# Wangshihu12/Voxel-SLAM

Hardware: AMD Instinct MI355X
Metric: local-BA iterations/sec (200k pts, W=10) (higher is better)
Workload: dtype f64

## Files before the change

voxel-slam_amd/csrc/vba_kernels_factor.hpp:

```cpp
#pragma once
#include <hip/hip_runtime.h>
#include "vba_eig3.hpp"

namespace vba {

struct FactorView {
  double *cl;
  double *fix;
  double *coe;
  double *eigval;
  double *eigvec;
  double *pcr;
  unsigned int *occ;
  int *tiles;
  int vs;
  int W;
};

__host__ __device__ inline int mask_bucket(unsigned int m, int nb) {
  constexpr int C[11][11] = {{1, 0, 0, 0, 0, 0, 0, 0, 0, 0, 0}, {1, 1, 0, 0, 0, 0, 0, 0, 0, 0, 0}, {1, 2, 1, 0, 0, 0, 0, 0, 0, 0, 0}, {1, 3, 3, 1, 0, 0, 0, 0, 0, 0, 0},
                             {1, 4, 6, 4, 1, 0, 0, 0, 0, 0, 0}, {1, 5, 10, 10, 5, 1, 0, 0, 0, 0, 0}, {1, 6, 15, 20, 15, 6, 1, 0, 0, 0, 0},
                             {1, 7, 21, 35, 35, 21, 7, 1, 0, 0, 0}, {1, 8, 28, 56, 70, 56, 28, 8, 1, 0, 0}, {1, 9, 36, 84, 126, 126, 84, 36, 9, 1, 0},
                             {1, 10, 45, 120, 210, 252, 210, 120, 45, 10, 1}};
  int p = 0;
  for (int b = 0; b < nb; b++) p += (m >> b) & 1u;
  int off = 0;
  for (int q = nb; q > p; q--) off += C[nb][q];
  int r = 0, k = 0;
  for (int b = 0; b < nb; b++)
    if ((m >> b) & 1u) { k++; r += C[b][k]; }
  return off + r;
}

__device__ __forceinline__ void jacobi_rot(double &app, double &aqq, double &apq, double &arp, double &arq,
                                           double &v0p, double &v0q, double &v1p, double &v1q, double &v2p, double &v2q,
                                           int sweep) {
  if (apq == 0.0) return;
  const double g = 100.0 * fabs(apq);
  if (fabs(app) + g == fabs(app) && fabs(aqq) + g == fabs(aqq)) { apq = 0.0; return; }
  const double a = 0.5 * (aqq - app);
  int ex;
  (void)frexp(fmax(fabs(a), fabs(apq)), &ex);
  const float af = (float)ldexp(a, -ex), bf = (float)ldexp(apq, -ex);
  const float tf = bf * __builtin_amdgcn_rcpf(fabsf(af) + __builtin_amdgcn_sqrtf(af * af + bf * bf));
  const double t = (af < 0.0f) ? -(double)tf : (double)tf;
  const double x = 1.0 + t * t;
  double c = __builtin_amdgcn_rsq(x);
  c = c * (1.5 - 0.5 * x * c * c);
  c = c * (1.5 - 0.5 * x * c * c);
  const double s = t * c;
  const double cc = c * c, ss = s * s, cs = c * s;
  const double npp = cc * app - 2.0 * cs * apq + ss * aqq;
  const double nqq = ss * app + 2.0 * cs * apq + cc * aqq;
  const double npq = cs * (app - aqq) + (cc - ss) * apq;
  app = npp; aqq = nqq; apq = npq;
  double x1 = arp, y1 = arq;
  arp = c * x1 - s * y1; arq = s * x1 + c * y1;
  x1 = v0p; y1 = v0q; v0p = c * x1 - s * y1; v0q = s * x1 + c * y1;
  x1 = v1p; y1 = v1q; v1p = c * x1 - s * y1; v1q = s * x1 + c * y1;
  x1 = v2p; y1 = v2q; v2p = c * x1 - s * y1; v2q = s * x1 + c * y1;
}

#define VBA_SWAP(a, b) { double _t = a; a = b; b = _t; }

__device__ __forceinline__ Eig3 eig3_jacobi_dev(double a00, double a01, double a02, double a11, double a12, double a22) {
  int e = 0;
  {
    const double s = fmax(fmax(fmax(fabs(a00), fabs(a11)), fabs(a22)), fmax(fmax(fabs(a01), fabs(a02)), fabs(a12)));
    if (s > 0.0 && s <= 1.7976931348623157e308) (void)frexp(s, &e);
  }
  a00 = ldexp(a00, -e); a01 = ldexp(a01, -e); a02 = ldexp(a02, -e); a11 = ldexp(a11, -e); a12 = ldexp(a12, -e); a22 = ldexp(a22, -e);
  double v00 = 1, v01 = 0, v02 = 0, v10 = 0, v11 = 1, v12 = 0, v20 = 0, v21 = 0, v22 = 1;
#pragma unroll 1
  for (int sweep = 0; sweep < 30; sweep++) {
    if (fabs(a01) + fabs(a02) + fabs(a12) == 0.0) break;
    jacobi_rot(a00, a11, a01, a02, a12, v00, v01, v10, v11, v20, v21, sweep);
    jacobi_rot(a00, a22, a02, a01, a12, v00, v02, v10, v12, v20, v22, sweep);
    jacobi_rot(a11, a22, a12, a01, a02, v01, v02, v11, v12, v21, v22, sweep);
  }
  if (a11 < a00) { VBA_SWAP(a00, a11); VBA_SWAP(v00, v01); VBA_SWAP(v10, v11); VBA_SWAP(v20, v21); }
  if (a22 < a00) { VBA_SWAP(a00, a22); VBA_SWAP(v00, v02); VBA_SWAP(v10, v12); VBA_SWAP(v20, v22); }
  if (a22 < a11) { VBA_SWAP(a11, a22); VBA_SWAP(v01, v02); VBA_SWAP(v11, v12); VBA_SWAP(v21, v22); }
  Eig3 o;
  o.w0 = ldexp(a00, e); o.w1 = ldexp(a11, e); o.w2 = ldexp(a22, e);
  o.v00 = v00; o.v01 = v01; o.v02 = v02; o.v10 = v10; o.v11 = v11; o.v12 = v12; o.v20 = v20; o.v21 = v21; o.v22 = v22;
  return o;
}

__device__ __forceinline__ void eig3_sym_dev(double a00, double a01, double a02, double a11, double a12, double a22,
                                             double &w0, double &w1, double &w2, double *V) {
  Eig3 o;
  if (!eig3_direct(a00, a01, a02, a11, a12, a22, o)) o = eig3_jacobi_dev(a00, a01, a02, a11, a12, a22);
  w0 = o.w0; w1 = o.w1; w2 = o.w2;
  V[0] = o.v00; V[1] = o.v01; V[2] = o.v02; V[3] = o.v10; V[4] = o.v11; V[5] = o.v12; V[6] = o.v20; V[7] = o.v21; V[8] = o.v22;
}

__global__ void k_aos_to_soa(FactorView f, int base, int n, const double *__restrict__ clusters, const double *__restrict__ fix,
                             const double *__restrict__ coe, const double *__restrict__ eig_val, const double *__restrict__ eig_vec,
                             const double *__restrict__ pcr_add) {
  const int W = f.W;
  const int per = 10 * W + 10 + 1 + 3 + 9 + 10;
  const long long tot = (long long)n * per;
  for (long long t = (long long)blockIdx.x * blockDim.x + threadIdx.x; t < tot; t += (long long)gridDim.x * blockDim.x) {
    const int a = (int)(t / per);
    int j = (int)(t % per);
    const int v = base + a;
    if (j < 10 * W) {
      const int i = j / 10, fld = j % 10;
      f.cl[((size_t)fld * W + i) * f.vs + v] = clusters[((size_t)a * W + i) * 10 + fld];
      continue;
    }
    j -= 10 * W;
    if (j < 10) { f.fix[(size_t)j * f.vs + v] = fix[(size_t)a * 10 + j]; continue; }
    j -= 10;
    if (j < 1) { f.coe[v] = coe[a]; continue; }
    j -= 1;
    if (j < 3) { f.eigval[(size_t)j * f.vs + v] = eig_val[(size_t)a * 3 + j]; continue; }
    j -= 3;
    if (j < 9) { f.eigvec[(size_t)j * f.vs + v] = eig_vec[(size_t)a * 9 + j]; continue; }
    j -= 9;
    f.pcr[(size_t)j * f.vs + v] = pcr_add[(size_t)a * 10 + j];
  }
}

__global__ void k_soa_to_aos_out(FactorView f, int n, double *__restrict__ eig_val, double *__restrict__ eig_vec, double *__restrict__ pcr_add) {
  const long long tot = (long long)n * 22;
  for (long long t = (long long)blockIdx.x * blockDim.x + threadIdx.x; t < tot; t += (long long)gridDim.x * blockDim.x) {
    const int v = (int)(t / 22);
    int j = (int)(t % 22);
    if (j < 3) { eig_val[(size_t)v * 3 + j] = f.eigval[(size_t)j * f.vs + v]; continue; }
    j -= 3;
    if (j < 9) { eig_vec[(size_t)v * 9 + j] = f.eigvec[(size_t)j * f.vs + v]; continue; }
    j -= 9;
    pcr_add[(size_t)v * 10 + j] = f.pcr[(size_t)j * f.vs + v];
  }
}

__global__ void k_factor_mask(FactorView f, int base, int n) {
  const int t = blockIdx.x * blockDim.x + threadIdx.x;
  if (t >= n) return;
  const int v = base + t;
  const size_t vs = (size_t)f.vs;
  unsigned int m = 0;
  for (int i = 0; i < f.W; i++) m |= (f.cl[((size_t)9 * f.W + i) * vs + v] != 0.0) ? (1u << i) : 0u;
  f.occ[v] = m;
}

__global__ void k_count_slots(FactorView f, int n, unsigned long long *out) {
  const long long tot = (long long)n * f.W;
  unsigned long long c = 0;
  for (long long t = (long long)blockIdx.x * blockDim.x + threadIdx.x; t < tot; t += (long long)gridDim.x * blockDim.x) {
    const int i = (int)(t / n), v = (int)(t % n);
    if (f.cl[((size_t)9 * f.W + i) * f.vs + v] != 0.0) c++;
  }
  if (c) atomicAdd(out, c);
}

__global__ __launch_bounds__(256) void k_calib_read8(const double *__restrict__ buf, double *__restrict__ sink) {
  const size_t nthr = (size_t)gridDim.x * blockDim.x, t = (size_t)blockIdx.x * blockDim.x + threadIdx.x;
  double acc = 0.0;
#pragma unroll
  for (int k = 0; k < 16; k++) acc += buf[t + (size_t)k * nthr];
  if (acc == 123.456) sink[0] = acc;
}

struct Cl10 { double p00, p10, p20, p11, p21, p22, v0, v1, v2, n; };
__device__ __forceinline__ Cl10 cluster_transform_exact(double c0, double c1, double c2, double c3, double c4, double c5, double v0, double v1, double v2, double n,
                                                        const double *R) {
#pragma clang fp contract(off)
  const double R0 = R[0], R1 = R[1], R2 = R[2], R3 = R[3], R4 = R[4], R5 = R[5], R6 = R[6], R7 = R[7], R8 = R[8];
  const double tx = R[9], ty = R[10], tz = R[11];
  const double rv0 = (R0 * v0 + R1 * v1) + R2 * v2, rv1 = (R3 * v0 + R4 * v1) + R5 * v2, rv2 = (R6 * v0 + R7 * v1) + R8 * v2;
  const double m00 = (R0 * c0 + R1 * c1) + R2 * c2, m01 = (R0 * c1 + R1 * c3) + R2 * c4, m02 = (R0 * c2 + R1 * c4) + R2 * c5;
  const double m10 = (R3 * c0 + R4 * c1) + R5 * c2, m11 = (R3 * c1 + R4 * c3) + R5 * c4, m12 = (R3 * c2 + R4 * c4) + R5 * c5;
  const double m20 = (R6 * c0 + R7 * c1) + R8 * c2, m21 = (R6 * c1 + R7 * c3) + R8 * c4, m22 = (R6 * c2 + R7 * c4) + R8 * c5;
  Cl10 o;
  o.p00 = ((((m00 * R0 + m01 * R1) + m02 * R2) + rv0 * tx) + rv0 * tx) + (tx * tx) * n;
  o.p10 = ((((m10 * R0 + m11 * R1) + m12 * R2) + rv1 * tx) + rv0 * ty) + (ty * tx) * n;
  o.p20 = ((((m20 * R0 + m21 * R1) + m22 * R2) + rv2 * tx) + rv0 * tz) + (tz * tx) * n;
  o.p11 = ((((m10 * R3 + m11 * R4) + m12 * R5) + rv1 * ty) + rv1 * ty) + (ty * ty) * n;
  o.p21 = ((((m20 * R3 + m21 * R4) + m22 * R5) + rv2 * ty) + rv1 * tz) + (tz * ty) * n;
  o.p22 = ((((m20 * R6 + m21 * R7) + m22 * R8) + rv2 * tz) + rv2 * tz) + (tz * tz) * n;
  o.v0 = rv0 + tx * n; o.v1 = rv1 + ty * n; o.v2 = rv2 + tz * n;
  o.n = n;
  return o;
}

__device__ __forceinline__ double wave_sum(double x) {
  for (int m = 32; m >= 1; m >>= 1) x += __shfl_xor(x, m, 64);
  return x;
}

__device__ __forceinline__ double dpp_mov_f64(double x, double old, const int ctrl, const int row_mask) {
  const long long xi = __double_as_longlong(x), oi = __double_as_longlong(old);
  int lo = (int)xi, hi = (int)(xi >> 32);
  const int olo = (int)oi, ohi = (int)(oi >> 32);
  switch (ctrl) {
    case 0xB1: lo = __builtin_amdgcn_update_dpp(olo, lo, 0xB1, 0xF, 0xF, false); hi = __builtin_amdgcn_update_dpp(ohi, hi, 0xB1, 0xF, 0xF, false); break;
    case 0x4E: lo = __builtin_amdgcn_update_dpp(olo, lo, 0x4E, 0xF, 0xF, false); hi = __builtin_amdgcn_update_dpp(ohi, hi, 0x4E, 0xF, 0xF, false); break;
    case 0x141: lo = __builtin_amdgcn_update_dpp(olo, lo, 0x141, 0xF, 0xF, false); hi = __builtin_amdgcn_update_dpp(ohi, hi, 0x141, 0xF, 0xF, false); break;
    case 0x140: lo = __builtin_amdgcn_update_dpp(olo, lo, 0x140, 0xF, 0xF, false); hi = __builtin_amdgcn_update_dpp(ohi, hi, 0x140, 0xF, 0xF, false); break;
    case 0x142: lo = __builtin_amdgcn_update_dpp(olo, lo, 0x142, 0xA, 0xF, false); hi = __builtin_amdgcn_update_dpp(ohi, hi, 0x142, 0xA, 0xF, false); break;
    default: lo = __builtin_amdgcn_update_dpp(olo, lo, 0x143, 0xC, 0xF, false); hi = __builtin_amdgcn_update_dpp(ohi, hi, 0x143, 0xC, 0xF, false); break;
  }
  (void)row_mask;
  return __longlong_as_double(((long long)hi << 32) | (unsigned int)lo);
}
__device__ __forceinline__ double group8_sum(double x) {
  x += dpp_mov_f64(x, x, 0xB1, 0xF);
  x += dpp_mov_f64(x, x, 0x4E, 0xF);
  x += dpp_mov_f64(x, x, 0x141, 0xF);
  return x;
}
__device__ __forceinline__ double wave_sum_to_lane63(double x) {
  x += dpp_mov_f64(x, x, 0xB1, 0xF);
  x += dpp_mov_f64(x, x, 0x4E, 0xF);
  x += dpp_mov_f64(x, x, 0x141, 0xF);
  x += dpp_mov_f64(x, x, 0x140, 0xF);
  x += dpp_mov_f64(x, 0.0, 0x142, 0xA);
  x += dpp_mov_f64(x, 0.0, 0x143, 0xC);
  return x;
}

template <int W, int TV>
struct ResCfg {
  static constexpr int NT = ((TV * W + 63) / 64) * 64;
  static constexpr int NF = NT / TV;
  static constexpr int KPT = (10 + NF - 1) / NF;
  static_assert(TV <= 64 && (TV & (TV - 1)) == 0 && NT % TV == 0, "the voxel threads are the first TV lanes of wave 0");
  static_assert(W * 12 <= NT, "one thread per pose scalar");
};

template <int W, int TV, bool STAMPS>
__global__ __launch_bounds__((ResCfg<W, TV>::NT)) void k_residual_s(FactorView f, const double *__restrict__ poses, int head, int end,
                                                                  double *__restrict__ partial, const int *__restrict__ gate,
                                                                  long long *__restrict__ stamps) {
  using C = ResCfg<W, TV>;
  __shared__ double T[10][W][TV];
  __shared__ double S[10][TV];
  __shared__ double sp[W * 12];
  const int gate_v = gate ? *gate : 1;
  const int tid = threadIdx.x, vl = tid % TV, fi = tid / TV;
  const int v = head + blockIdx.x * TV + vl;
  const size_t vs = (size_t)f.vs, fs = (size_t)W * vs;
  const int vc = v < end ? v : end - 1;
  const int fic = fi < W ? fi : W - 1;
  long long st0 = 0, st1 = 0, st2 = 0, st3 = 0;
  if (STAMPS) st0 = clock64();
  const unsigned int occm = f.occ[vc];
  const double pose_s = poses[tid < W * 12 ? tid : 0];
  double acc[C::KPT];
#pragma unroll
  for (int j = 0; j < C::KPT; j++) { const int k = fi + j * C::NF; acc[j] = f.fix[(size_t)(k < 10 ? k : 9) * vs + vc]; }
  double coe = f.coe[vc];
  unsigned int occv = occm;
  asm volatile("" : "+v"(occv), "+v"(coe), "+v"(acc[0]));
  if (gate_v == 0) return;
  if (tid < W * 12) sp[tid] = pose_s;
  const bool occ = fi < W && v < end && ((occv >> fic) & 1u);
  double c[9], n = 0.0;
#pragma unroll
  for (int k = 0; k < 9; k++) c[k] = occ ? f.cl[(size_t)k * fs + (size_t)fi * vs + v] : 0.0;
  if (occ) n = f.cl[9 * fs + (size_t)fi * vs + v];
  __syncthreads();
  if (occ) {
    const Cl10 w = cluster_transform_exact(c[0], c[1], c[2], c[3], c[4], c[5], c[6], c[7], c[8], n, sp + 12 * fi);
    T[0][fi][vl] = w.p00; T[1][fi][vl] = w.p10; T[2][fi][vl] = w.p20; T[3][fi][vl] = w.p11; T[4][fi][vl] = w.p21; T[5][fi][vl] = w.p22;
    T[6][fi][vl] = w.v0; T[7][fi][vl] = w.v1; T[8][fi][vl] = w.v2;
    T[9][fi][vl] = n;
  } else if (fi < W) {
#pragma unroll
    for (int k = 0; k < 10; k++) T[k][fi][vl] = 0.0;
  }
  __syncthreads();
#pragma unroll
  for (int j = 0; j < C::KPT; j++) {
    const int k = fi + j * C::NF;
    if (k < 10) {
      double a = acc[j];
#pragma unroll
      for (int i = 0; i < W; i++) a += T[k][i][vl];
      S[k][vl] = a;
      if (v < end) f.pcr[(size_t)k * vs + v] = a;
    }
  }
  __syncthreads();
  if (STAMPS) st1 = clock64();
  double r = 0.0;
  if (fi == 0 && v < end) {
    const double Nv = S[9][vl];
    double iN = __builtin_amdgcn_rcp(Nv);
    iN = iN * (2.0 - Nv * iN);
    iN = iN * (2.0 - Nv * iN);
    const double b0 = S[6][vl] * iN, b1 = S[7][vl] * iN, b2 = S[8][vl] * iN;
    double w0, w1, w2, V[9];
    eig3_sym_dev(S[0][vl] * iN - b0 * b0, S[1][vl] * iN - b1 * b0, S[2][vl] * iN - b2 * b0, S[3][vl] * iN - b1 * b1, S[4][vl] * iN - b2 * b1,
                 S[5][vl] * iN - b2 * b2, w0, w1, w2, V);
    if (STAMPS) st2 = clock64();
    f.eigval[0 * vs + v] = w0; f.eigval[1 * vs + v] = w1; f.eigval[2 * vs + v] = w2;
#pragma unroll
    for (int k = 0; k < 9; k++) f.eigvec[(size_t)k * vs + v] = V[k];
    r = coe * w0;
  }
  if (tid < 64) {
    r = wave_sum_to_lane63(r);
    if (tid == 63) partial[blockIdx.x] = r;
    if (STAMPS && tid == 0 && blockIdx.x < 2048) {
      st3 = clock64();
      long long *o = stamps + (size_t)blockIdx.x * 4;
      o[0] = st0; o[1] = st1; o[2] = st2; o[3] = st3;
    }
  }
}

template <int W, bool STAMPS>
__global__ __launch_bounds__(64) void k_residual_v(FactorView f, const double *__restrict__ poses, int head, int end,
                                                   double *__restrict__ partial, const int *__restrict__ gate, long long *__restrict__ stamps) {
  const int gate_v = gate ? *gate : 1;
  const int lane = threadIdx.x;
  const int v = head + blockIdx.x * 64 + lane;
  const size_t vs = (size_t)f.vs, fs = (size_t)W * vs;
  const int vc = v < end ? v : end - 1;
  long long st0 = 0, st1 = 0, st2 = 0, st3 = 0;
  if (STAMPS) st0 = clock64();
  unsigned int occm = f.occ[vc];
  double acc[10];
#pragma unroll
  for (int k = 0; k < 10; k++) acc[k] = f.fix[(size_t)k * vs + vc];
  double coe = f.coe[vc];
  asm volatile("" : "+v"(occm), "+v"(coe), "+v"(acc[0]));
  if (gate_v == 0) return;
  if (v >= end) occm = 0;
  double c[W][10];
#pragma unroll
  for (int i = 0; i < W; i++) {
    const bool on = (occm >> i) & 1u;
    if (__ballot(on) != 0ull) {
#pragma unroll
      for (int k = 0; k < 10; k++) c[i][k] = on ? f.cl[(size_t)k * fs + (size_t)i * vs + v] : 0.0;
    } else {
#pragma unroll
      for (int k = 0; k < 10; k++) c[i][k] = 0.0;
    }
  }
#pragma unroll
  for (int i = 0; i < W; i++) {
    const bool on = (occm >> i) & 1u;
    if (__ballot(on) != 0ull) {
      if (on) {
        const Cl10 w = cluster_transform_exact(c[i][0], c[i][1], c[i][2], c[i][3], c[i][4], c[i][5], c[i][6], c[i][7], c[i][8], c[i][9], poses + 12 * i);
        acc[0] += w.p00; acc[1] += w.p10; acc[2] += w.p20; acc[3] += w.p11; acc[4] += w.p21; acc[5] += w.p22;
        acc[6] += w.v0; acc[7] += w.v1; acc[8] += w.v2; acc[9] += w.n;
      }
    }
  }
  if (STAMPS) st1 = clock64();
  double r = 0.0;
  if (v < end) {
#pragma unroll
    for (int k = 0; k < 10; k++) f.pcr[(size_t)k * vs + v] = acc[k];
    const double Nv = acc[9];
    double iN = __builtin_amdgcn_rcp(Nv);
    iN = iN * (2.0 - Nv * iN);
    iN = iN * (2.0 - Nv * iN);
    const double b0 = acc[6] * iN, b1 = acc[7] * iN, b2 = acc[8] * iN;
    double w0, w1, w2, V[9];
    eig3_sym_dev(acc[0] * iN - b0 * b0, acc[1] * iN - b1 * b0, acc[2] * iN - b2 * b0, acc[3] * iN - b1 * b1, acc[4] * iN - b2 * b1,
                 acc[5] * iN - b2 * b2, w0, w1, w2, V);
    if (STAMPS) st2 = clock64();
    f.eigval[0 * vs + v] = w0; f.eigval[1 * vs + v] = w1; f.eigval[2 * vs + v] = w2;
#pragma unroll
    for (int k = 0; k < 9; k++) f.eigvec[(size_t)k * vs + v] = V[k];
    r = coe * w0;
  }
  r = wave_sum_to_lane63(r);
  if (lane == 63) partial[blockIdx.x] = r;
  if (STAMPS && lane == 0 && blockIdx.x < 2048) {
    st3 = clock64();
    long long *o = stamps + (size_t)blockIdx.x * 4;
    o[0] = st0; o[1] = st1; o[2] = st2; o[3] = st3;
  }
}

__global__ __launch_bounds__(256) void k_reduce_partials(const double *__restrict__ partial, int nb, int nout, double *__restrict__ out,
                                                        const int *__restrict__ gate) {
  __shared__ double s[256];
  const int gate_v = gate ? *gate : 1;
  const int j = threadIdx.x & 15, q = threadIdx.x >> 4;
  const int o = blockIdx.x * 16 + j, oc = o < nout ? o : nout - 1;
  double pv[16];
#pragma unroll
  for (int k = 0; k < 16; k++) { const int b = q + 16 * k; pv[k] = partial[(size_t)(b < nb ? b : 0) * nout + oc]; }
#pragma unroll
  for (int k = 0; k < 16; k++) asm volatile("" : "+v"(pv[k]));
  if (gate_v == 0) return;
  double acc = 0.0;
  if (o < nout) {
#pragma unroll
    for (int k = 0; k < 16; k++) acc += (q + 16 * k < nb) ? pv[k] : 0.0;
    for (int b = q + 256; b < nb; b += 16) acc += partial[(size_t)b * nout + o];
  }
  s[threadIdx.x] = acc;
  __syncthreads();
  if (q == 0 && o < nout) {
    double t = 0.0;
#pragma unroll
    for (int k = 0; k < 16; k++) t += s[16 * k + j];
    out[o] = t;
  }
}

__global__ __launch_bounds__(256) void k_sum_scalar(const double *__restrict__ partial, int nb, double *__restrict__ out,
                                                   const int *__restrict__ gate) {
  __shared__ double s[4];
  if (gate && *gate == 0) return;
  double acc = 0.0;
  for (int b = threadIdx.x; b < nb; b += 256) acc += partial[b];
  acc = wave_sum(acc);
  if ((threadIdx.x & 63) == 0) s[threadIdx.x >> 6] = acc;
  __syncthreads();
  if (threadIdx.x == 0) out[0] = (s[0] + s[1]) + (s[2] + s[3]);
}

typedef double v4f64 __attribute__((ext_vector_type(4)));

constexpr int hess2_tv(int W) {
  return W == 2 ? 128 : W == 3 ? 80 : W == 4 ? 64 : W == 5 ? 48 : W == 6 ? 40 : (W == 7 || W == 8) ? 32 : (W == 9 || W == 10) ? 24 : 16;
}
constexpr int gcd_i(int a, int b) { return b == 0 ? a : gcd_i(b, a % b); }

__device__ __forceinline__ double rcp_f64(double x) {
  double y = __builtin_amdgcn_rcp(x);
  y = y * (2.0 - x * y);
  y = y * (2.0 - x * y);
  return y;
}

template <int W>
struct HessCfg2 {
  static constexpr int TV = hess2_tv(W);
  static constexpr int NT = 256;
  static constexpr int NC = 6 * W;
  static constexpr int NT16 = (NC + 15) / 16;
  static constexpr int NCP = 16 * NT16;
  static constexpr int GS = ((NCP % 32 == 16) ? NCP : NCP + 16) + 1;
  static constexpr int NK = 3 * TV;
  static constexpr int NWV = NT / 64;
  static constexpr int NU = NT16 * (NT16 + 1) / 2;
  static constexpr int KS = NWV / gcd_i(NU, NWV);
  static constexpr int UPW = NU * KS / NWV;
  static constexpr int KSTEPS = NK / 4 / KS;
  static constexpr int NOUT = NC * NC + NC + 1;
  static constexpr int EB = NU * 256;
  static constexpr int GB = EB + 21 * W;
  static constexpr int RB = GB + 6 * W;
  static constexpr int NOUT2 = RB + 1;
  static constexpr int NG8 = NT / 8;
  static_assert(TV * W <= NT && TV % 8 == 0 && (NK / 4) % KS == 0 && (NU * KS) % NWV == 0, "tile shape");
  static constexpr bool PRESCALE = ((size_t)2 * NK * GS + NK + W * 12 + 8) * sizeof(double) <= (size_t)150 * 1024;
  static constexpr size_t LDS_MAIN = (size_t)NK * GS * (PRESCALE ? 2 : 1) + NK + W * 12 + 8;
  static constexpr size_t LDS_EPI = (size_t)(KS > 1 ? NU * 256 : 0) + (size_t)28 * NG8 + 8;
  static constexpr size_t LDS_BYTES = (LDS_MAIN > LDS_EPI ? LDS_MAIN : LDS_EPI) * sizeof(double);
};

struct SlotLoad {
  double n, c[9], coe, l0, l1, l2, NN, vs0, vs1, vs2, U[9];
  bool valid;
};

template <int W>
__device__ __forceinline__ void slot_load(const FactorView &f, int v, int fi, int end, unsigned int occm, SlotLoad &q) {
  const size_t vs = (size_t)f.vs, fs = (size_t)W * vs;
  q.valid = v < end;
  if (q.valid) {
    const double *cp = f.cl + (size_t)fi * vs + v;
    const bool on = (occm >> fi) & 1u;
    q.n = on ? cp[9 * fs] : 0.0;
#pragma unroll
    for (int k = 0; k < 9; k++) q.c[k] = on ? cp[(size_t)k * fs] : 0.0;
    q.coe = f.coe[v];
    q.l0 = f.eigval[v]; q.l1 = f.eigval[vs + v]; q.l2 = f.eigval[2 * vs + v];
    q.NN = f.pcr[9 * vs + v]; q.vs0 = f.pcr[6 * vs + v]; q.vs1 = f.pcr[7 * vs + v]; q.vs2 = f.pcr[8 * vs + v];
#pragma unroll
    for (int k = 0; k < 9; k++) q.U[k] = f.eigvec[(size_t)k * vs + v];
  }
}

__device__ __forceinline__ void slot_terms(const SlotLoad &q, const double *R, bool first, double *g1, double *g2, double *hh, double &ck1, double &ck2, double &ck3,
                                           double *Err, double *Ert, double *Ett, double *gj, double &rres) {
if (q.valid) {
  const double coe = q.coe, l0 = q.l0, NN = q.NN;
  const double inn = rcp_f64(NN);
  const double c1 = 2.0 * rcp_f64(l0 - q.l1), c2 = 2.0 * rcp_f64(l0 - q.l2);
  ck1 = coe * c1; ck2 = coe * c2; ck3 = coe * (-2.0 * inn * inn);
  if (first) rres += coe * l0;
  const double n = q.n;
  if (n != 0.0) {
    const double pxx = q.c[0], pxy = q.c[1], pxz = q.c[2], pyy = q.c[3], pyz = q.c[4], pzz = q.c[5];
    const double vx = q.c[6], vy = q.c[7], vz = q.c[8];
    const double u00 = q.U[0], u01 = q.U[1], u02 = q.U[2], u10 = q.U[3], u11 = q.U[4], u12 = q.U[5], u20 = q.U[6], u21 = q.U[7], u22 = q.U[8];
    const double bx = q.vs0 * inn, by = q.vs1 * inn, bz = q.vs2 * inn;
    
    const double k0 = u00, k1 = u10, k2 = u20;
    const double a00 = R[0] * k0 + R[3] * k1 + R[6] * k2, a01 = R[1] * k0 + R[4] * k1 + R[7] * k2, a02 = R[2] * k0 + R[5] * k1 + R[8] * k2;
    const double a10 = R[0] * u01 + R[3] * u11 + R[6] * u21, a11 = R[1] * u01 + R[4] * u11 + R[7] * u21, a12 = R[2] * u01 + R[5] * u11 + R[8] * u21;
    const double a20 = R[0] * u02 + R[3] * u12 + R[6] * u22, a21 = R[1] * u02 + R[4] * u12 + R[7] * u22, a22 = R[2] * u02 + R[5] * u12 + R[8] * u22;
    const double tx = R[9] - bx, ty = R[10] - by, tz = R[11] - bz;
    const double s0 = k0 * tx + k1 * ty + k2 * tz, s1 = u01 * tx + u11 * ty + u21 * tz, s2 = u02 * tx + u12 * ty + u22 * tz;
    const double pa00 = pxx * a00 + pxy * a01 + pxz * a02, pa01 = pxy * a00 + pyy * a01 + pyz * a02, pa02 = pxz * a00 + pyz * a01 + pzz * a02;
    const double pa10 = pxx * a10 + pxy * a11 + pxz * a12, pa11 = pxy * a10 + pyy * a11 + pyz * a12, pa12 = pxz * a10 + pyz * a11 + pzz * a12;
    const double pa20 = pxx * a20 + pxy * a21 + pxz * a22, pa21 = pxy * a20 + pyy * a21 + pyz * a22, pa22 = pxz * a20 + pyz * a21 + pzz * a22;
    const double wx = pa00 + s0 * vx, wy = pa01 + s0 * vy, wz = pa02 + s0 * vz;
    const double c2x = R[0] * vx + R[1] * vy + R[2] * vz + n * tx;
    const double c2y = R[3] * vx + R[4] * vy + R[5] * vz + n * ty;
    const double c2z = R[6] * vx + R[7] * vy + R[8] * vz + n * tz;
    const double qx = vy * a02 - vz * a01, qy = vz * a00 - vx * a02, qz = vx * a01 - vy * a00;
    const double d0 = c2x * k0 + c2y * k1 + c2z * k2;
    const double d1 = c2x * u01 + c2y * u11 + c2z * u21;
    const double d2 = c2x * u02 + c2y * u12 + c2z * u22;
    const double j0 = 2.0 * (wy * a02 - wz * a01) * inn, j1 = 2.0 * (wz * a00 - wx * a02) * inn, j2 = 2.0 * (wx * a01 - wy * a00) * inn;
    const double j3 = 2.0 * d0 * k0 * inn, j4 = 2.0 * d0 * k1 * inn, j5 = 2.0 * d0 * k2 * inn;
    gj[0] += coe * j0; gj[1] += coe * j1; gj[2] += coe * j2; gj[3] += coe * j3; gj[4] += coe * j4; gj[5] += coe * j5;
    {
      const double bx1 = pa10 + s1 * vx, by1 = pa11 + s1 * vy, bz1 = pa12 + s1 * vz;
      g1[0] = (-(a01 * bz1 - a02 * by1) + (wy * a12 - wz * a11)) * inn;
      g1[1] = (-(a02 * bx1 - a00 * bz1) + (wz * a10 - wx * a12)) * inn;
      g1[2] = (-(a00 * by1 - a01 * bx1) + (wx * a11 - wy * a10)) * inn;
      g1[3] = (k0 * d1 + d0 * u01) * inn; g1[4] = (k1 * d1 + d0 * u11) * inn; g1[5] = (k2 * d1 + d0 * u21) * inn;
      const double bx2 = pa20 + s2 * vx, by2 = pa21 + s2 * vy, bz2 = pa22 + s2 * vz;
      g2[0] = (-(a01 * bz2 - a02 * by2) + (wy * a22 - wz * a21)) * inn;
      g2[1] = (-(a02 * bx2 - a00 * bz2) + (wz * a20 - wx * a22)) * inn;
      g2[2] = (-(a00 * by2 - a01 * bx2) + (wx * a21 - wy * a20)) * inn;
      g2[3] = (k0 * d2 + d0 * u02) * inn; g2[4] = (k1 * d2 + d0 * u12) * inn; g2[5] = (k2 * d2 + d0 * u22) * inn;
    }
    hh[0] = qx; hh[1] = qy; hh[2] = qz; hh[3] = n * k0; hh[4] = n * k1; hh[5] = n * k2;
    const double wa = wx * a00 + wy * a01 + wz * a02;
    const double t00 = a01 * pxz - a02 * pxy, t10 = a02 * pxx - a00 * pxz, t20 = a00 * pxy - a01 * pxx;
    const double t01 = a01 * pyz - a02 * pyy, t11 = a02 * pxy - a00 * pyz, t21 = a00 * pyy - a01 * pxy;
    const double t02 = a01 * pzz - a02 * pyz, t12 = a02 * pxz - a00 * pzz, t22 = a00 * pyz - a01 * pxz;
    const double S00 = t01 * a02 - t02 * a01, S01 = -t00 * a02 + t02 * a00, S02 = t00 * a01 - t01 * a00;
    const double S11 = -t10 * a02 + t12 * a00, S12 = t10 * a01 - t11 * a00;
    const double S22 = t20 * a01 - t21 * a00;
    const double e2 = 2.0 * inn * coe;
    Err[0] += e2 * (a00 * wx - wa - S00);
    Err[1] += e2 * (0.5 * (a00 * wy + wx * a01) - S01);
    Err[2] += e2 * (0.5 * (a00 * wz + wx * a02) - S02);
    Err[3] += e2 * (a01 * wy - wa - S11);
    Err[4] += e2 * (0.5 * (a01 * wz + wy * a02) - S12);
    Err[5] += e2 * (a02 * wz - wa - S22);
    Ert[0] += e2 * qx * k0; Ert[1] += e2 * qx * k1; Ert[2] += e2 * qx * k2;
    Ert[3] += e2 * qy * k0; Ert[4] += e2 * qy * k1; Ert[5] += e2 * qy * k2;
    Ert[6] += e2 * qz * k0; Ert[7] += e2 * qz * k1; Ert[8] += e2 * qz * k2;
    const double e3 = e2 * n;
    Ett[0] += e3 * k0 * k0; Ett[1] += e3 * k0 * k1; Ett[2] += e3 * k0 * k2; Ett[3] += e3 * k1 * k1; Ett[4] += e3 * k1 * k2; Ett[5] += e3 * k2 * k2;
  }
}
}

struct LmDev;
__device__ int lm_prev_stop(const LmDev *s);
__device__ double lm_r1(const LmDev *s);
__device__ const double *lm_xt(const LmDev *s);
__device__ void lm_update_apply(LmDev *s, double r2, int W);
__device__ __forceinline__ double lm_sum_partials(const double *__restrict__ r2_dev, int nb, int lane) {
  double pv[8];
#pragma unroll
  for (int k = 0; k < 8; k++) { const int b = lane + 64 * k; pv[k] = r2_dev[(nb > 0 && b < nb) ? b : 0]; }
  double acc = 0.0;
#pragma unroll
  for (int k = 0; k < 8; k++) acc += (lane + 64 * k < nb) ? pv[k] : 0.0;
  for (int b = lane + 512; b < nb; b += 64) acc += r2_dev[b];
  for (int m = 32; m >= 1; m >>= 1) acc += __shfl_xor(acc, m, 64);
  return acc;
}

struct LiDev;
struct LiJob { const LmDev *lm; LiDev *dev; const double *imu; double *himu, *gimu; };
__device__ void li_imu_body(const LmDev *s, LiDev *li, const double *imu, double *himu, double *gimu, double *lds);

template <int W>
__global__ __launch_bounds__(HessCfg2<W>::NT) void k_hessian2(FactorView f, const double *__restrict__ poses, int head, int end,
                                                             int ntiles, double *__restrict__ partial, const int *__restrict__ gate,
                                                             long long *__restrict__ stamps, LmDev *lm, const double *__restrict__ k4_partial, int k4_nb,
                                                             int nwg, LiJob li) {
  using C = HessCfg2<W>;
  extern __shared__ __attribute__((aligned(16))) double lds[];
  if (li.dev && blockIdx.x == 0) {
    li_imu_body(li.lm, li.dev, li.imu, li.himu, li.gimu, lds);
    return;
  }
  const int bid = (int)blockIdx.x - (li.dev ? 1 : 0);
  const int tile0 = (int)(((long long)bid * ntiles) / nwg), tile1 = (int)(((long long)(bid + 1) * ntiles) / nwg);
  const int my_vl = threadIdx.x % HessCfg2<W>::TV, my_fi = threadIdx.x / HessCfg2<W>::TV;
  unsigned int occ_nx = 0;
  if (my_fi < W && tile0 < tile1) { const int v0 = head + tile0 * HessCfg2<W>::TV + my_vl; occ_nx = f.occ[v0 < end ? v0 : end - 1]; }
  __shared__ int lm_dec[2];
  int gate_v = (gate && !lm) ? *gate : 1;
  double lm_r2 = 0.0;
  if (lm) {
    if (threadIdx.x < 64) {
      lm_r2 = lm_sum_partials(k4_partial, k4_nb, threadIdx.x);
      if (threadIdx.x == 0) {
        const double r1 = lm_r1(lm);
        const int stop = lm_prev_stop(lm);
        const bool accept = (r1 - lm_r2) > 0, nstop = fabs((r1 - lm_r2) / r1) < 1e-6;
        lm_dec[0] = (!stop && accept && !nstop) ? 1 : 0;
        lm_dec[1] = stop;
      }
    }
    poses = lm_xt(lm);
  }
#define VBA_STAMP(i) do { if (stamps && threadIdx.x == 0) stamps[(size_t)bid * 16 + (i)] = wall_clock64(); } while (0)
  VBA_STAMP(0);
  double *G = lds;
  double *GA = C::PRESCALE ? G + (size_t)C::NK * C::GS : G;
  double *cK = GA + (size_t)C::NK * C::GS;
  double *sp = cK + C::NK;
  const int tid = threadIdx.x, lane = tid & 63, wv = tid >> 6;

  for (int t = tid; t < W * 12; t += C::NT) sp[t] = poses[t];
  constexpr int PADC = C::GS - C::NC;
  if constexpr (PADC > 0)
    for (int t = tid; t < C::NK * PADC; t += C::NT) { G[(size_t)(t / PADC) * C::GS + C::NC + t % PADC] = 0.0; if (C::PRESCALE) GA[(size_t)(t / PADC) * C::GS + C::NC + t % PADC] = 0.0; }

  const int vl = tid % C::TV, fi = tid / C::TV;
  const bool slot_thread = fi < W;
  v4f64 acc[C::UPW];
#pragma unroll
  for (int t = 0; t < C::UPW; t++) acc[t] = (v4f64){0.0, 0.0, 0.0, 0.0};
  double Err[6] = {0, 0, 0, 0, 0, 0}, Ert[9] = {0, 0, 0, 0, 0, 0, 0, 0, 0}, Ett[6] = {0, 0, 0, 0, 0, 0};
  double gj[6] = {0, 0, 0, 0, 0, 0};
  double rres = 0.0;

  SlotLoad nx;
  nx.valid = false;
  if (slot_thread && tile0 < tile1) slot_load<W>(f, head + tile0 * C::TV + vl, fi, end, occ_nx, nx);
  if (slot_thread && tile0 + 1 < tile1) { const int v1 = head + (tile0 + 1) * C::TV + vl; occ_nx = f.occ[v1 < end ? v1 : end - 1]; }
  asm volatile("" : "+v"(nx.n));
  if (gate_v == 0) return;
  __syncthreads();
  if (lm) {
    const int run = lm_dec[0], was_stopped = lm_dec[1];
    if (bid == 0 && threadIdx.x < 64 && !was_stopped) lm_update_apply(lm, lm_r2, W);
    if (!run) return;
  }
  VBA_STAMP(1);
  int stamp_i = 2;

  for (int tile = tile0; tile < tile1; tile++) {
    if (slot_thread) {
      const SlotLoad q = nx;
      double g1[6] = {0, 0, 0, 0, 0, 0}, g2[6] = {0, 0, 0, 0, 0, 0}, hh[6] = {0, 0, 0, 0, 0, 0};
      double ck1 = 0.0, ck2 = 0.0, ck3 = 0.0;
      slot_terms(q, sp + 12 * fi, fi == 0, g1, g2, hh, ck1, ck2, ck3, Err, Ert, Ett, gj, rres);
      double *g = G + (size_t)(3 * vl) * C::GS + 6 * fi;
#pragma unroll
      for (int d = 0; d < 6; d++) { g[d] = g1[d]; g[C::GS + d] = g2[d]; g[2 * C::GS + d] = hh[d]; }
      if (C::PRESCALE) {
        double *ga = GA + (size_t)(3 * vl) * C::GS + 6 * fi;
#pragma unroll
        for (int d = 0; d < 6; d++) { ga[d] = g1[d] * ck1; ga[C::GS + d] = g2[d] * ck2; ga[2 * C::GS + d] = hh[d] * ck3; }
      }
      if (fi == 0) { cK[3 * vl] = ck1; cK[3 * vl + 1] = ck2; cK[3 * vl + 2] = ck3; }
      const int nt = tile + 1;
      nx.valid = false;
      if (nt < tile1) {
        slot_load<W>(f, head + nt * C::TV + vl, fi, end, occ_nx, nx);
        if (nt + 1 < tile1) { const int v2 = head + (nt + 1) * C::TV + vl; occ_nx = f.occ[v2 < end ? v2 : end - 1]; }
      }
    }
    __syncthreads();
    if (stamp_i < 12) { VBA_STAMP(stamp_i); stamp_i++; }
    {
      const int kr = lane >> 4, cl = lane & 15;
      const double *gap[C::UPW], *gbp[C::UPW], *ckp[C::UPW];
#pragma unroll
      for (int t = 0; t < C::UPW; t++) {
        const int unit = wv * C::UPW + t;
        const int u = unit % C::NU, ksp = unit / C::NU;
        int p = u, ta = 0;
        while (p >= C::NT16 - ta) { p -= C::NT16 - ta; ta++; }
        const int tb = ta + p;
        const int kb = ksp * C::KSTEPS * 4;
        gap[t] = GA + (size_t)(kb + kr) * C::GS + 16 * ta + cl;
        gbp[t] = G + (size_t)(kb + kr) * C::GS + 16 * tb + cl;
        ckp[t] = cK + kb + kr;
      }
      double ar[C::UPW], cr[C::UPW], br[C::UPW];
#pragma unroll
      for (int t = 0; t < C::UPW; t++) { ar[t] = gap[t][0]; cr[t] = C::PRESCALE ? 1.0 : ckp[t][0]; br[t] = gbp[t][0]; }
#pragma unroll
      for (int ks = 0; ks < C::KSTEPS; ks++) {
        double av[C::UPW], bv[C::UPW];
#pragma unroll
        for (int t = 0; t < C::UPW; t++) { av[t] = C::PRESCALE ? ar[t] : ar[t] * cr[t]; bv[t] = br[t]; }
        if (ks + 1 < C::KSTEPS) {
          const int k = 4 * (ks + 1);
#pragma unroll
          for (int t = 0; t < C::UPW; t++) { ar[t] = gap[t][(size_t)k * C::GS]; if (!C::PRESCALE) cr[t] = ckp[t][k]; br[t] = gbp[t][(size_t)k * C::GS]; }
        }
        __builtin_amdgcn_sched_barrier(0);
#pragma unroll
        for (int t = 0; t < C::UPW; t++) acc[t] = __builtin_amdgcn_mfma_f64_16x16x4f64(av[t], bv[t], acc[t], 0, 0, 0);
        __builtin_amdgcn_sched_barrier(0);
      }
    }
    __syncthreads();
    if (stamp_i < 12) { VBA_STAMP(stamp_i); stamp_i++; }
  }
  VBA_STAMP(12);

  double *out = partial + (size_t)bid * C::NOUT2;
  double *Tb = lds;
  double *Eb = Tb + (C::KS > 1 ? C::NU * 256 : 0);
  if (C::KS > 1) {
#pragma unroll
    for (int t = 0; t < C::UPW; t++) {
      const int unit = wv * C::UPW + t;
      if (unit / C::NU != 0) {
        const int u = unit % C::NU;
#pragma unroll
        for (int r = 0; r < 4; r++) {
          if (unit / C::NU == 1) Tb[u * 256 + r * 64 + lane] = acc[t][r];
        }
      }
    }
    for (int ksp = 2; ksp < C::KS; ksp++) {
      __syncthreads();
#pragma unroll
      for (int t = 0; t < C::UPW; t++) {
        const int unit = wv * C::UPW + t;
        if (unit / C::NU == ksp) {
          const int u = unit % C::NU;
#pragma unroll
          for (int r = 0; r < 4; r++) Tb[u * 256 + r * 64 + lane] += acc[t][r];
        }
      }
    }
  }
#pragma unroll
  for (int k = 0; k < 6; k++) { Err[k] = group8_sum(Err[k]); Ett[k] = group8_sum(Ett[k]); gj[k] = group8_sum(gj[k]); }
#pragma unroll
  for (int k = 0; k < 9; k++) Ert[k] = group8_sum(Ert[k]);
  rres = group8_sum(rres);
  if ((tid & 7) == 0) {
    const int g8 = tid >> 3;
#pragma unroll
    for (int k = 0; k < 6; k++) { Eb[(size_t)k * C::NG8 + g8] = Err[k]; Eb[(size_t)(15 + k) * C::NG8 + g8] = Ett[k]; Eb[(size_t)(21 + k) * C::NG8 + g8] = gj[k]; }
#pragma unroll
    for (int k = 0; k < 9; k++) Eb[(size_t)(6 + k) * C::NG8 + g8] = Ert[k];
    Eb[(size_t)27 * C::NG8 + g8] = rres;
  }
  __syncthreads();
  VBA_STAMP(13);
#pragma unroll
  for (int t = 0; t < C::UPW; t++) {
    const int unit = wv * C::UPW + t;
    if (unit / C::NU == 0) {
      const int u = unit % C::NU;
#pragma unroll
      for (int r = 0; r < 4; r++) {
        double val = acc[t][r];
        if (C::KS > 1) val += Tb[u * 256 + r * 64 + lane];
        out[u * 256 + r * 64 + lane] = val;
      }
    }
  }
  for (int t = tid; t < 28 * W; t += C::NT) {
    const int k = t % 28, fr = t / 28;
    double sum = 0.0;
#pragma unroll
    for (int g = 0; g < C::TV / 8; g++) sum += Eb[(size_t)k * C::NG8 + fr * (C::TV / 8) + g];
    if (k < 21) out[C::EB + 21 * fr + k] = sum;
    else if (k < 27) out[C::GB + 6 * fr + (k - 21)] = sum;
    else if (fr == 0) out[C::RB] = sum;
  }
  VBA_STAMP(14);
#undef VBA_STAMP
}

template <int W>
__device__ __forceinline__ double tl_fetch(const double *__restrict__ red, int row, int col) {
  using C = HessCfg2<W>;
  if (row > col) { const int t = row; row = col; col = t; }
  const int ta = row >> 4, tb = col >> 4;
  const int u = ta * C::NT16 - ta * (ta - 1) / 2 + (tb - ta);
  const int rt = row & 15, ct = col & 15;
  double val = red[u * 256 + (rt >> 2) * 64 + (rt & 3) * 16 + ct];
  const int fr = row / 6;
  if (col / 6 == fr) {
    const int a = row - 6 * fr, b = col - 6 * fr;
    int idx;
    if (b < 3) idx = a * 3 - a * (a - 1) / 2 + (b - a);
    else if (a < 3) idx = 6 + 3 * a + (b - 3);
    else { const int a2 = a - 3, b2 = b - 3; idx = 15 + a2 * 3 - a2 * (a2 - 1) / 2 + (b2 - a2); }
    val += red[C::EB + 21 * fr + idx];
  }
  return val;
}

template <int W>
__global__ void k_tiles_to_full(const double *__restrict__ red, double *__restrict__ full) {
  using C = HessCfg2<W>;
  for (int t = blockIdx.x * blockDim.x + threadIdx.x; t < C::NOUT; t += gridDim.x * blockDim.x) {
    if (t < C::NC * C::NC) full[t] = tl_fetch<W>(red, t / C::NC, t % C::NC);
    else if (t < C::NC * C::NC + C::NC) full[t] = red[C::GB + (t - C::NC * C::NC)];
    else full[t] = red[C::RB];
  }
}

}
```

voxel-slam_amd/csrc/vba_kernels_lm.hpp:

```cpp
#pragma once
#include <hip/hip_runtime.h>
#include "vba_ldlt.hpp"

namespace vba {

constexpr int LM_SPEC = 4;

struct LmDev {
  double x[VBA_MAX_WIN_DEV * 12];
  double xt[VBA_MAX_WIN_DEV * 12];
  double u, v, r1, r2, q1, resis_first;
  int is_calc_hess, stop, iter, n_trace, all_accepted, last_accepted, max_trace, run_hess, run_res, pad;
  double trace[5 * 64];
  long long stamps[64];
  int spec_n, spec_i, use_spec, pad2;
  double q1_spec[LM_SPEC];
  double xt_spec[LM_SPEC][VBA_MAX_WIN_DEV * 12];
};

__device__ __forceinline__ void so3_exp_dev(const double *w, double *R) {
  const double n = sqrt(w[0] * w[0] + w[1] * w[1] + w[2] * w[2]);
  if (n >= 1e-11) {
    const double a0 = w[0] / n, a1 = w[1] / n, a2 = w[2] / n;
    const double s = sin(n), c1 = 1.0 - cos(n);
    R[0] = 1.0 + c1 * (a0 * a0 - 1.0); R[1] = -s * a2 + c1 * a0 * a1;    R[2] = s * a1 + c1 * a0 * a2;
    R[3] = s * a2 + c1 * a1 * a0;      R[4] = 1.0 + c1 * (a1 * a1 - 1.0); R[5] = -s * a0 + c1 * a1 * a2;
    R[6] = -s * a1 + c1 * a2 * a0;     R[7] = s * a0 + c1 * a2 * a1;     R[8] = 1.0 + c1 * (a2 * a2 - 1.0);
  } else {
    R[0] = 1; R[1] = 0; R[2] = 0; R[3] = 0; R[4] = 1; R[5] = 0; R[6] = 0; R[7] = 0; R[8] = 1;
  }
}



template <int W>
__host__ __device__ __forceinline__ int tl_eidx(int row, int col) {
  using C = HessCfg2<W>;
  const int fr = row / 6;
  if (col / 6 != fr) return -1;
  const int a = row - 6 * fr, b = col - 6 * fr;
  int idx;
  if (b < 3) idx = a * 3 - a * (a - 1) / 2 + (b - a);
  else if (a < 3) idx = 6 + 3 * a + (b - 3);
  else { const int a2 = a - 3, b2 = b - 3; idx = 15 + a2 * 3 - a2 * (a2 - 1) / 2 + (b2 - a2); }
  return C::EB + 21 * fr + idx;
}

template <int W, bool COPY_RAW>
__global__ __launch_bounds__(256) void k_lm_solve_m(LmDev *s, const double *__restrict__ red, double *__restrict__ raw, double *__restrict__ dx_out) {
  const int sb = blockIdx.x;
  using C2 = HessCfg2<W>;
  constexpr int n = 6 * W, NT = 256, NP = ((n + 1 + 15) / 16) * 16, NH = (n + 63) / 64, NU = C2::NU, T16 = C2::NT16;
  using LC = LdltCfg<NP>;
  constexpr int IMG = NP * (NP + 1) / 2, ZERO = (n + 1) * (n + 2) / 2;
  static_assert(IMG <= LC::LTOT && NP >= n + 2, "the image must lie in the L region: ldlt_mfma writes P while the tiles are read");
  __shared__ __attribute__((aligned(16))) double lds[LC::DOUBLES];
  __shared__ double hd[n], gs[n], xs[NP], dxs[n], red8[8];
  __shared__ int ord[n];
  double *Lst = lds, *Tp = Lst + LC::LTOT, *P = Tp + NP * LC::LS, *img = lds;
  const int tid = threadIdx.x, lane = tid & 63, wv = tid >> 6;
  const int use_spec = s->use_spec, stop = s->stop, calc = s->is_calc_hess;
  const double u0 = s->u, v0 = s->v;
  __builtin_amdgcn_sched_barrier(0);
  double dgt[NH], dge[NH], gv[NH];
  auto load_diag = [&](const double *__restrict__ src) {
#pragma unroll
    for (int h = 0; h < NH; h++) {
      const int k = lane + 64 * h, kc = k < n ? k : n - 1, ta = kc >> 4, rt = kc & 15;
      dgt[h] = src[(ta * T16 - ta * (ta - 1) / 2) * 256 + (rt >> 2) * 64 + (rt & 3) * 16 + rt];
      dge[h] = src[tl_eidx<W>(kc, kc)];
      gv[h] = src[C2::GB + kc];
    }
  };
  const int ru = (lane >> 4) + 4 * wv, cu = lane & 15;
  double tv[NU], ev[NU];
  bool eon[NU];
  auto load_bulk = [&](const double *__restrict__ src) {
    int u = 0;
#pragma unroll
    for (int ta = 0; ta < T16; ta++)
#pragma unroll
      for (int tb = ta; tb < T16; tb++, u++) {
        const int row = 16 * ta + ru, col = 16 * tb + cu;
        const int e = (row <= col && col < n) ? tl_eidx<W>(row, col) : -1;
        eon[u] = e >= 0;
        tv[u] = src[u * 256 + tid];
        ev[u] = src[e >= 0 ? e : C2::EB];
      }
  };
  if constexpr (!COPY_RAW) { load_diag(red); load_bulk(red); }
  const double r_v = COPY_RAW ? 0.0 : red[C2::RB];
  double xr[12];
  if (wv == 3 && lane < W)
#pragma unroll
    for (int k = 0; k < 12; k++) xr[k] = s->x[12 * lane + k];
  const long long t_begin = clock64();
  if (stop || use_spec) return;
  double u = u0;
  { double vb = v0; for (int k = 0; k < sb; k++) { u = u * vb; vb = 2 * vb; } }
  if constexpr (COPY_RAW) {
    const double *__restrict__ src = calc ? red : raw;
    if (calc && sb == 0)
      for (int t = tid; t < C2::NOUT2; t += NT) raw[t] = src[t];
    load_diag(src); load_bulk(src);
  }
  double hk[NH], dk[NH];
  int rk[NH];
#pragma unroll
  for (int h = 0; h < NH; h++) {
    const int k = lane + 64 * h;
    hk[h] = k < 6 ? 1.0 : dgt[h] + dge[h];
    dk[h] = fabs(hk[h] + u * hk[h]);
    rk[h] = 0;
  }
#pragma unroll
  for (int j = 0; j < n; j++) {
    const double o = readlane_f64(dk[j >> 6], j & 63);
#pragma unroll
    for (int h = 0; h < NH; h++) rk[h] += (o > dk[h] || (o == dk[h] && j < lane + 64 * h)) ? 1 : 0;
  }
  int prow[T16], pcol[T16];
#pragma unroll
  for (int t = 0; t < T16; t++) {
    const int r = 16 * t + ru, c = 16 * t + cu;
    prow[t] = __shfl(rk[(16 * t) >> 6], (r < n ? r : n - 1) & 63);
    pcol[t] = __shfl(rk[(16 * t) >> 6], (c < n ? c : n - 1) & 63);
  }
  {
    int uu = 0;
#pragma unroll
    for (int ta = 0; ta < T16; ta++)
#pragma unroll
      for (int tb = ta; tb < T16; tb++, uu++) {
        const int row = 16 * ta + ru, col = 16 * tb + cu;
        if (row <= col && col < n) {
          double a = eon[uu] ? tv[uu] + ev[uu] : tv[uu];
          a = (row < 6) ? ((row == col) ? 1.0 : 0.0) : a;
          a = (row == col) ? a + u * a : a;
          const int pr = prow[ta], pc = pcol[tb], hi = pr > pc ? pr : pc, lo = pr > pc ? pc : pr;
          img[hi * (hi + 1) / 2 + lo] = a;
        }
      }
  }
  if (wv == 0)
#pragma unroll
    for (int h = 0; h < NH; h++) {
      const int k = lane + 64 * h;
      if (k < n) {
        const double g = k < 6 ? 0.0 : gv[h];
        hd[k] = hk[h]; gs[k] = g; ord[rk[h]] = k;
        img[n * (n + 1) / 2 + rk[h]] = -g;
      }
    }
#pragma unroll
  for (int i = n; i < NP; i++)
    if (tid <= i && (i > n || tid >= n)) img[i * (i + 1) / 2 + tid] = (tid == i) ? 1.0 : 0.0;
  const int iter0 = s->iter, dbg = s->pad;
  if (tid == 0 && calc && sb == 0) { const double r = COPY_RAW ? red[C2::RB] : r_v; s->r1 = r; if (iter0 == 0) s->resis_first = r; }
  long long *stamps = ((dbg & 16) && tid == 0 && sb == 0) ? s->stamps : nullptr;
  if (stamps) stamps[0] = t_begin;
  __syncthreads();
  auto elem = [&](int i, int j) -> double {
    return img[i >= j ? i * (i + 1) / 2 + j : ZERO];
  };
  if (stamps) stamps[1] = clock64();
  ldlt_mfma<NP, NT>(Lst, Tp, P, n, elem, ((dbg & 16) && sb == 0) ? s->stamps : nullptr);
  if (stamps) stamps[3] = clock64();
  if (tid < n) xs[tid] = Lst[LC::lat(n, tid)];
  __syncthreads();
  const double x = ldlt_backsub<NP>(Lst, xs, n);
  if (stamps) stamps[4] = clock64();
  if (tid < n) dxs[ord[tid]] = x;
  __syncthreads();
  if (wv == 3) {
    if (lane < W) {
      double E[9];
      so3_exp_dev(dxs + 6 * lane, E);
      const double *R = xr;
      double *Rt = (sb == 0 ? s->xt : s->xt_spec[sb]) + 12 * lane;
#pragma unroll
      for (int r = 0; r < 3; r++)
#pragma unroll
        for (int c = 0; c < 3; c++) Rt[3 * r + c] = R[3 * r] * E[c] + R[3 * r + 1] * E[3 + c] + R[3 * r + 2] * E[6 + c];
#pragma unroll
      for (int k = 0; k < 3; k++) Rt[9 + k] = R[9 + k] + dxs[6 * lane + 3 + k];
    }
    if (lane == 63) red8[3] = 0.0;
  } else {
    double q = tid < n ? dxs[tid] * (u * hd[tid] * dxs[tid] - gs[tid]) : 0.0;
    q = wave_sum_to_lane63(q);
    if (lane == 63) red8[wv] = q;
  }
  __syncthreads();
  if (dx_out && tid < n) dx_out[sb * n + tid] = dxs[tid];
  if (tid == 0) {
    const double q1 = 0.5 * (red8[0] + red8[1] + red8[2] + red8[3]);
    s->q1_spec[sb] = q1;
    if (sb == 0) { s->q1 = q1; s->spec_n = gridDim.x; s->spec_i = 0; }
  }
  if (stamps) stamps[5] = clock64();
}


__device__ int lm_prev_stop(const LmDev *s) { return s->stop; }
__device__ double lm_r1(const LmDev *s) { return s->r1; }
__device__ const double *lm_xt(const LmDev *s) { return s->xt; }

__device__ void lm_update_apply(LmDev *s, double r2, int W) {
  const int ntr = s->n_trace, mtr = s->max_trace, it = s->iter, spec_n = s->spec_n, spec_nx = s->spec_i + 1;
  const double r1 = s->r1, q1 = s->q1, u0 = s->u, v0 = s->v;
  const int lane = threadIdx.x & 63;
  const bool have_spec = spec_nx < spec_n;
  const double *xs_ = s->xt_spec[have_spec ? spec_nx : 0];
  double sp0 = 0.0, sp1 = 0.0, sp2 = 0.0;
  if (have_spec) {
    if (lane < 12 * W) sp0 = xs_[lane];
    if (lane + 64 < 12 * W) sp1 = xs_[lane + 64];
    if (lane + 128 < 12 * W) sp2 = xs_[lane + 128];
  }
  const double q1_nx = s->q1_spec[have_spec ? spec_nx : 0];
  double xt0 = 0.0, xt1 = 0.0, xt2 = 0.0;
  if (lane < 12 * W) xt0 = s->xt[lane];
  if (lane + 64 < 12 * W) xt1 = s->xt[lane + 64];
  if (lane + 128 < 12 * W) xt2 = s->xt[lane + 128];
  double q = r1 - r2, u = u0, v = v0;
  const bool accept = q > 0;
  if (accept) {
    if (lane < 12 * W) s->x[lane] = xt0;
    if (lane + 64 < 12 * W) s->x[lane + 64] = xt1;
    if (lane + 128 < 12 * W) s->x[lane + 128] = xt2;
    const double one_three = 1.0 / 3;
    q = q / q1;
    v = 2;
    const double t = 2 * q - 1;
    q = 1 - t * t * t;
    u *= (q < one_three ? one_three : q);
  } else {
    u = u * v;
    v = 2 * v;
    if (have_spec) {
      if (lane < 12 * W) s->xt[lane] = sp0;
      if (lane + 64 < 12 * W) s->xt[lane + 64] = sp1;
      if (lane + 128 < 12 * W) s->xt[lane + 128] = sp2;
    }
  }
  if (lane != 0) return;
  if (!accept && have_spec) { s->q1 = q1_nx; s->spec_i = spec_nx; s->use_spec = 1; }
  else { s->use_spec = 0; s->spec_n = 0; }
  s->r2 = r2;
  if (ntr < mtr) {
    double *t = s->trace + 5 * ntr;
    t[0] = r1; t[1] = r2; t[2] = u0; t[3] = v0; t[4] = q1;
    s->n_trace = ntr + 1;
  }
  s->u = u; s->v = v;
  s->is_calc_hess = accept ? 1 : 0;
  s->last_accepted = accept ? 1 : 0;
  if (!accept) s->all_accepted = 0;
  s->iter = it + 1;
  const int nstop = (fabs((r1 - r2) / r1) < 1e-6) ? 1 : 0;
  s->stop = nstop;
  s->run_res = nstop ? 0 : 1;
  s->run_hess = (accept && !nstop) ? 1 : 0;
}

__global__ __launch_bounds__(64) void k_lm_update(LmDev *s, const double *__restrict__ r2_dev, int nb, int W) {
  const int stop = s->stop;
  const double r2 = (nb > 0) ? lm_sum_partials(r2_dev, nb, threadIdx.x) : r2_dev[0];
  if (stop) return;
  lm_update_apply(s, r2, W);
}

}
```

voxel-slam_amd/csrc/voxelba.hip:

```cpp
#include "../../include/voxelba.h"

#define VBA_MAX_WIN_DEV VBA_MAX_WIN
#include "vba_kernels_factor.hpp"
#include "vba_kernels_h3.hpp"
#include "vba_kernels_map.hpp"
#include "vba_kernels_lm.hpp"
#include "vba_kernels_li.hpp"
#include "vba_kernels_scan.hpp"
#include "vba_kernels_gba.hpp"
#include "vba_kernels_big.hpp"
#include "vba_kernels_pgo.hpp"
#include "vba_kernels_kd.hpp"
#include "vba_kernels_init.hpp"
#include "vba_kernels_btc.hpp"
#include "vba_btcgen.hpp"
#include "vba_io.hpp"
#include <cstddef>
#include "vba_hostmath.hpp"

#include <hip/hip_runtime.h>
#include <rccl/rccl.h>
#include <dlfcn.h>
#include <cstdio>
#include <cstdlib>
#include <cstring>
#include <atomic>
#include <string>
#include <thread>
#include <vector>
#include <array>
#include <map>
#include <chrono>
#include <deque>
#include <functional>
#include <algorithm>

using namespace vba;

#define HIPCHK(ctx, expr)                                                                        \
  do {                                                                                           \
    hipError_t _e = (expr);                                                                      \
    if (_e != hipSuccess) {                                                                      \
      (ctx)->set_error(std::string(#expr) + ": " + hipGetErrorString(_e));                       \
      return VBA_ERR_HIP;                                                                        \
    }                                                                                            \
  } while (0)

namespace {
struct TimedSpan { hipEvent_t a, b; };

struct RcclApi {
  ncclResult_t (*GetUniqueId)(ncclUniqueId *) = nullptr;
  ncclResult_t (*CommInitRank)(ncclComm_t *, int, ncclUniqueId, int) = nullptr;
  ncclResult_t (*CommDestroy)(ncclComm_t) = nullptr;
  ncclResult_t (*AllReduce)(const void *, void *, size_t, ncclDataType_t, ncclRedOp_t, ncclComm_t, hipStream_t) = nullptr;
  ncclResult_t (*AllGather)(const void *, void *, size_t, ncclDataType_t, ncclComm_t, hipStream_t) = nullptr;
  const char *(*GetErrorString)(ncclResult_t) = nullptr;
  bool ok = false;
  std::string why;
};
const RcclApi &rccl_api() {
  static const RcclApi api = [] {
    RcclApi a;
    void *h = nullptr;
    if (dlsym(RTLD_DEFAULT, "ncclAllReduce")) h = RTLD_DEFAULT;
    if (!h) h = dlopen("librccl.so.1", RTLD_NOW | RTLD_LOCAL);
    if (!h) h = dlopen("librccl.so", RTLD_NOW | RTLD_LOCAL);
    if (!h) h = dlopen("/opt/rocm/lib/librccl.so.1", RTLD_NOW | RTLD_LOCAL);
    if (!h) { const char *e = dlerror(); a.why = std::string("librccl.so.1 not found: ") + (e ? e : "?"); return a; }
    bool all = true;
    auto get = [&](const char *name) { void *s = dlsym(h, name); if (!s) { all = false; a.why = std::string("RCCL lacks ") + name; } return s; };
    a.GetUniqueId = (decltype(a.GetUniqueId))get("ncclGetUniqueId");
    a.CommInitRank = (decltype(a.CommInitRank))get("ncclCommInitRank");
    a.CommDestroy = (decltype(a.CommDestroy))get("ncclCommDestroy");
    a.AllReduce = (decltype(a.AllReduce))get("ncclAllReduce");
    a.AllGather = (decltype(a.AllGather))get("ncclAllGather");
    a.GetErrorString = (decltype(a.GetErrorString))get("ncclGetErrorString");
    a.ok = all;
    return a;
  }();
  return api;
}

inline const char *diag_env(const char *name) {
#ifdef VBA_DIAG
  return std::getenv(name);
#else
  (void)name;
  return nullptr;
#endif
}
}

struct vba_ctx {
  vba_options opt;
  int device = 0;
  hipStream_t stream = nullptr;
  bool own_stream = false;
  std::string err;

  FactorView fv{};
  int nvox = 0;
  int nvox_global = 0;
  int cap = 0;
  double *d_poses = nullptr;
  double *d_partial = nullptr;
  size_t partial_doubles = 0;
  double *d_out = nullptr;
  double *d_full = nullptr;
  double *d_scal = nullptr;
  double *h_pin = nullptr;
  size_t pin_doubles = 0;
  void *d_stage = nullptr;
  size_t stage_bytes = 0;

  vba_allreduce_fn allreduce = nullptr;
  void *allreduce_user = nullptr;
  int rank = 0, n_ranks = 1;
  bool force_collective = false;
  int max_blocks_hess = 256;
  int residual_vpl_from = 45000;
  bool use_h3 = false;
  ncclComm_t comm = nullptr;
  bool own_comm = false;
  bool collective_off = false;
  bool collective() const { return !collective_off && (allreduce || comm) && (n_ranks > 1 || force_collective); }

  bool timing = false;
  std::string timing_only;
  int timing_every = 1; unsigned timing_ctr = 0;
  int lm_spec = LM_SPEC;
  std::vector<std::array<double, 450>> covinv_cache; size_t covinv_next = 0;
  std::map<std::string, std::vector<TimedSpan>> spans;

  LmDev *d_lm = nullptr;
  LmDev *h_lm = nullptr;
  static const int kLmRing = 8;
  LmDev *h_lm_up[kLmRing] = {nullptr};
  hipEvent_t lm_up_ev[kLmRing] = {nullptr};
  int lm_up_next = 0;
  double *d_raw = nullptr;
  struct { bool active = false; int thd_num = 2; bool have_hess = false; bool pending_update = false; int k4_nb = 0; } lm;
  int k4part_cap = 0;
  double *d_k4part = nullptr;
  std::vector<double> trace;

  LiDev *d_li = nullptr;
  double *d_imu = nullptr, *d_himu = nullptr, *d_gimu = nullptr;

  MapStore map;
  GbaStore gba;
  BigStore big;
  double *d_kdtree[2] = {nullptr, nullptr};
  size_t kd_cap = 0; int kd_n = 0, kd_cur = 0;
  double *d_refpts = nullptr;
  size_t refpts_doubles = 0;
  double *d_lipack = nullptr; size_t lipack_doubles = 0;
  double *d_liscr = nullptr; size_t liscr_doubles = 0;
  double *d_hba_all = nullptr; size_t hba_all_doubles = 0;
  std::vector<vba_ctx *> hba_workers;
  void *d_init = nullptr; size_t init_bytes = 0;
  char *d_btcq = nullptr, *h_btcq = nullptr; size_t btcq_bytes = 0;
  int *d_btccnt = nullptr; size_t btccnt_cap = 0;
  BtcIcpDev *d_icp = nullptr, *h_icp = nullptr;
  unsigned long long *d_icpkey = nullptr; size_t icpkey_cap = 0;
  double *d_icppart = nullptr; size_t icppart_cap = 0;
  char *d_pgo = nullptr; size_t pgo_bytes = 0;
  double *d_pgoAb = nullptr; size_t pgoAb_bytes = 0;
  static const int kExpRing = 4;
  char *h_exp[kExpRing] = {nullptr}; hipEvent_t exp_ev[kExpRing] = {nullptr}; int exp_next = 0;
  char *d_exp = nullptr; size_t exp_cap = 0;
  char *d_expout = nullptr; size_t expout_cap = 0;
  std::vector<long long> exp_first; std::vector<int> exp_kbase;

  void set_error(const std::string &s) { err = s; }
};

namespace {

static const int kMaxDevices = 64;
static const int kMaxBlocksHess = 256;

int nout_of(int W) { return 36 * W * W + 6 * W + 1; }
int nout_tl(int W) {
  const int nt16 = (6 * W + 15) / 16;
  return nt16 * (nt16 + 1) / 2 * 256 + 27 * W + 1;
}

static inline bool span_on(vba_ctx *c, const char *name) { return c->timing && (c->timing_only.empty() || c->timing_only == name); }
void span_begin(vba_ctx *c, const char *name, TimedSpan &s) {
  s.a = s.b = nullptr;
  if (!span_on(c, name)) return;
  if (c->timing_every > 1 && (c->timing_ctr++ % c->timing_every) != 0) return;
  hipEventCreate(&s.a); hipEventCreate(&s.b);
  hipEventRecord(s.a, c->stream);
}
void span_end(vba_ctx *c, const char *name, TimedSpan &s) {
  if (!s.a) return;
  hipEventRecord(s.b, c->stream);
  c->spans[name].push_back(s);
}

int ensure_pin(vba_ctx *c, size_t n) {
  if (n <= c->pin_doubles) return VBA_OK;
  if (c->h_pin) hipHostFree(c->h_pin);
  c->h_pin = nullptr; c->pin_doubles = 0;
  HIPCHK(c, hipHostMalloc((void **)&c->h_pin, n * sizeof(double), hipHostMallocDefault));
  c->pin_doubles = n;
  return VBA_OK;
}
int ensure_stage(vba_ctx *c, size_t bytes) {
  if (bytes <= c->stage_bytes) return VBA_OK;
  if (c->d_stage) hipFree(c->d_stage);
  c->d_stage = nullptr; c->stage_bytes = 0;
  HIPCHK(c, hipMalloc(&c->d_stage, bytes));
  c->stage_bytes = bytes;
  return VBA_OK;
}

int factor_reserve(vba_ctx *c, int need) {
  if (need <= c->cap) return VBA_OK;
  int newcap = c->cap ? c->cap : 4096;
  while (newcap < need) newcap *= 2;
  newcap = (newcap + 63) / 64 * 64 + 64 * 33;
  const int W = c->opt.win_size;
  FactorView n = c->fv;
  n.vs = newcap; n.W = W;
  const size_t rows[6] = {(size_t)10 * W, 10, 1, 3, 9, 10};
  double **np[6] = {&n.cl, &n.fix, &n.coe, &n.eigval, &n.eigvec, &n.pcr};
  double *op[6] = {c->fv.cl, c->fv.fix, c->fv.coe, c->fv.eigval, c->fv.eigvec, c->fv.pcr};
  for (int k = 0; k < 6; k++) {
    HIPCHK(c, hipMalloc((void **)np[k], rows[k] * newcap * sizeof(double)));
    HIPCHK(c, hipMemsetAsync(*np[k], 0, rows[k] * newcap * sizeof(double), c->stream));
    if (c->nvox > 0 && op[k])
      HIPCHK(c, hipMemcpy2DAsync(*np[k], (size_t)newcap * sizeof(double), op[k], (size_t)c->cap * sizeof(double),
                                 (size_t)c->nvox * sizeof(double), rows[k], hipMemcpyDeviceToDevice, c->stream));
  }
  unsigned int *oocc = c->fv.occ;
  int *otiles = c->fv.tiles;
  HIPCHK(c, hipMalloc((void **)&n.tiles, ((size_t)4 * newcap + 16) * sizeof(int)));
  HIPCHK(c, hipMemsetAsync(n.tiles, 0, ((size_t)4 * newcap + 16) * sizeof(int), c->stream));
  HIPCHK(c, hipMalloc((void **)&n.occ, (size_t)newcap * sizeof(unsigned int)));
  HIPCHK(c, hipMemsetAsync(n.occ, 0, (size_t)newcap * sizeof(unsigned int), c->stream));
  if (c->nvox > 0 && oocc) HIPCHK(c, hipMemcpyAsync(n.occ, oocc, (size_t)c->nvox * sizeof(unsigned int), hipMemcpyDeviceToDevice, c->stream));
  HIPCHK(c, hipStreamSynchronize(c->stream));
  for (int k = 0; k < 6; k++) if (op[k]) hipFree(op[k]);
  if (oocc) hipFree(oocc);
  if (otiles) hipFree(otiles);
  c->fv = n;
  if (c->nvox > 0 && c->use_h3) hipLaunchKernelGGL(k_factor_tiles, dim3(1), dim3(1024), 0, c->stream, c->fv, c->nvox);
  c->cap = newcap;
  return VBA_OK;
}

void factor_update_mask(vba_ctx *c, int base, int n) {
  if (n > 0) hipLaunchKernelGGL(k_factor_mask, dim3((n + 255) / 256), dim3(256), 0, c->stream, c->fv, base, n);
  if (base + n > 0 && c->use_h3) hipLaunchKernelGGL(k_factor_tiles, dim3(1), dim3(1024), 0, c->stream, c->fv, base + n);
}

int upload_poses(vba_ctx *c, const double *poses) {
  const int W = c->opt.win_size;
  int st = ensure_pin(c, 65536);
  if (st) return st;
  std::memcpy(c->h_pin, poses, (size_t)W * 12 * sizeof(double));
  HIPCHK(c, hipMemcpyAsync(c->d_poses, c->h_pin, (size_t)W * 12 * sizeof(double), hipMemcpyHostToDevice, c->stream));
  return VBA_OK;
}

template <int W>
int launch_hessian2_t(vba_ctx *c, const double *poses_dev, const int *gate, int head, int end, int *nblocks_out, LmDev *lm, const double *k4p, int k4nb,
                      const LiJob &li, size_t li_lds) {
  using C = HessCfg2<W>;
  const int ntiles = (end - head + C::TV - 1) / C::TV;
  const int maxb = li.dev ? c->max_blocks_hess - 1 : c->max_blocks_hess;
  int nb = ntiles < maxb ? ntiles : maxb;
  if (nb < 1) nb = 1;
  static bool attr_set[kMaxDevices] = {false};
  if (!attr_set[c->device % kMaxDevices]) {
    const size_t li_max = 150 * 1024;
    hipFuncSetAttribute((const void *)k_hessian2<W>, hipFuncAttributeMaxDynamicSharedMemorySize, (int)(C::LDS_BYTES > li_max ? C::LDS_BYTES : li_max));
    attr_set[c->device % kMaxDevices] = true;
  }
  long long *stamps = nullptr;
  static const bool want_stamps = diag_env("VBA_K3_STAMPS") != nullptr;
  if (want_stamps) {
    static long long *d_st = nullptr;
    if (!d_st) hipMalloc((void **)&d_st, (size_t)kMaxBlocksHess * 16 * 8);
    hipMemsetAsync(d_st, 0, (size_t)kMaxBlocksHess * 16 * 8, c->stream);
    stamps = d_st;
  }
  const size_t lds = (li.dev && li_lds > C::LDS_BYTES) ? li_lds : C::LDS_BYTES;
  hipLaunchKernelGGL(k_hessian2<W>, dim3(nb + (li.dev ? 1 : 0)), dim3(C::NT), lds, c->stream, c->fv, poses_dev, head, end, ntiles, c->d_partial, gate, stamps, lm, k4p, k4nb,
                     nb, li);
  if (want_stamps) {
    std::vector<long long> h((size_t)nb * 16);
    hipStreamSynchronize(c->stream);
    hipMemcpy(h.data(), stamps, h.size() * 8, hipMemcpyDeviceToHost);
    long long t0 = h[0];
    for (int b = 0; b < nb; b++) if (h[(size_t)b * 16] && h[(size_t)b * 16] < t0) t0 = h[(size_t)b * 16];
    for (int b : {0, 1, nb / 2, nb - 1}) {
      fprintf(stderr, "[k3 stamps] wg %d:", b);
      for (int i = 0; i < 15; i++) fprintf(stderr, " %lld", h[(size_t)b * 16 + i] ? h[(size_t)b * 16 + i] - t0 : -1);
      fprintf(stderr, "\n");
    }
    long long tmax = 0;
    for (int b = 0; b < nb; b++) if (h[(size_t)b * 16 + 14] - t0 > tmax) tmax = h[(size_t)b * 16 + 14] - t0;
    fprintf(stderr, "[k3 stamps] last workgroup ends at %lld ticks (100 MHz wall clock: 1 tick = 10 ns)\n", tmax);
  }
  *nblocks_out = nb;
  return VBA_OK;
}

template <int W>
int launch_hessian3_t(vba_ctx *c, const double *poses_dev, const int *gate, int *nblocks_out, LmDev *lm, const double *k4p, int k4nb, const LiJob &li, size_t li_lds) {
  using C = HessCfg3<W>;
  const int nb = li.dev ? c->max_blocks_hess - 1 : c->max_blocks_hess;
  static bool attr_set[kMaxDevices] = {false};
  if (!attr_set[c->device % kMaxDevices]) {
    const size_t li_max = 150 * 1024;
    hipFuncSetAttribute((const void *)k_hessian3<W>, hipFuncAttributeMaxDynamicSharedMemorySize, (int)(C::LDS_BYTES > li_max ? C::LDS_BYTES : li_max));
    attr_set[c->device % kMaxDevices] = true;
  }
  const size_t lds = (li.dev && li_lds > C::LDS_BYTES) ? li_lds : C::LDS_BYTES;
  long long *stamps = nullptr;
  static const bool want_stamps = diag_env("VBA_K3_STAMPS") != nullptr;
  if (want_stamps) {
    static long long *d_st = nullptr;
    if (!d_st) hipMalloc((void **)&d_st, (size_t)kMaxBlocksHess * 16 * 8);
    hipMemsetAsync(d_st, 0, (size_t)kMaxBlocksHess * 16 * 8, c->stream);
    stamps = d_st;
  }
  hipLaunchKernelGGL(k_hessian3<W>, dim3(nb + (li.dev ? 1 : 0)), dim3(C::NT), lds, c->stream, c->fv, poses_dev, c->nvox, c->d_partial, gate, lm, k4p, k4nb, nb, li, stamps);
  if (want_stamps) {
    std::vector<long long> h((size_t)nb * 16);
    hipStreamSynchronize(c->stream);
    hipMemcpy(h.data(), stamps, h.size() * 8, hipMemcpyDeviceToHost);
    long long t0 = h[0];
    for (int b = 0; b < nb; b++) if (h[(size_t)b * 16] && h[(size_t)b * 16] < t0) t0 = h[(size_t)b * 16];
    for (int b : {0, 1, nb / 2, nb - 1}) {
      fprintf(stderr, "[k3 stamps] wg %d:", b);
      for (int i = 0; i < 16; i++) fprintf(stderr, " %lld", h[(size_t)b * 16 + i] ? h[(size_t)b * 16 + i] - t0 : -1);
      fprintf(stderr, "\n");
    }
    long long tmax = 0;
    for (int b = 0; b < nb; b++) if (h[(size_t)b * 16 + 15] - t0 > tmax) tmax = h[(size_t)b * 16 + 15] - t0;
    fprintf(stderr, "[k3 stamps] last workgroup ends at %lld ticks (100 MHz wall clock: 1 tick = 10 ns); per workgroup: start, prologue, then per tile [A, B, combine, E]\n", tmax);
  }
  *nblocks_out = nb;
  return VBA_OK;
}

int launch_hessian(vba_ctx *c, const double *pd, const int *gate, int head, int end, int *nb, LmDev *lm = nullptr, const double *k4p = nullptr, int k4nb = 0,
                   const LiJob &li = LiJob{}, size_t li_lds = 0) {
  if (head == 0 && end == c->nvox && c->opt.win_size <= 10 && c->use_h3) {
    switch (c->opt.win_size) {
#define VBA_H3_CASE(WW) case WW: return launch_hessian3_t<WW>(c, pd, gate, nb, lm, k4p, k4nb, li, li_lds);
      VBA_H3_CASE(2) VBA_H3_CASE(3) VBA_H3_CASE(4) VBA_H3_CASE(5) VBA_H3_CASE(6) VBA_H3_CASE(7) VBA_H3_CASE(8) VBA_H3_CASE(9) VBA_H3_CASE(10)
#undef VBA_H3_CASE
    }
  }
  switch (c->opt.win_size) {
#define VBA_H_CASE(WW) case WW: return launch_hessian2_t<WW>(c, pd, gate, head, end, nb, lm, k4p, k4nb, li, li_lds);
    VBA_H_CASE(2) VBA_H_CASE(3) VBA_H_CASE(4) VBA_H_CASE(5) VBA_H_CASE(6) VBA_H_CASE(7) VBA_H_CASE(8) VBA_H_CASE(9) VBA_H_CASE(10)
    VBA_H_CASE(11) VBA_H_CASE(12) VBA_H_CASE(13) VBA_H_CASE(14) VBA_H_CASE(15) VBA_H_CASE(16)
#undef VBA_H_CASE
    default: return VBA_ERR_UNSUPPORTED_WINDOW;
  }
}

#ifndef VBA_K4_TV
#define VBA_K4_TV 32
#endif
inline bool residual_vpl(const vba_ctx *c, int n) { return n > c->residual_vpl_from; }
inline int residual_nb(const vba_ctx *c, int n) { return residual_vpl(c, n) ? (n + 63) / 64 : (n + VBA_K4_TV - 1) / VBA_K4_TV; }

void k4_stamps_dump(vba_ctx *c, int nb, long long *d_st) {
  const int n = nb < 2048 ? nb : 2048;
  std::vector<long long> h((size_t)n * 4);
  hipStreamSynchronize(c->stream);
  hipMemcpy(h.data(), d_st, h.size() * 8, hipMemcpyDeviceToHost);
  long long t0 = h[0];
  for (int b = 0; b < n; b++) if (h[b * 4] && h[b * 4] < t0) t0 = h[b * 4];
  double a = 0, e = 0, w = 0, last = 0;
  for (int b = 0; b < n; b++) { a += h[b * 4 + 1] - h[b * 4]; e += h[b * 4 + 2] - h[b * 4 + 1]; w += h[b * 4 + 3] - h[b * 4 + 2]; if (h[b * 4 + 3] - t0 > last) last = h[b * 4 + 3] - t0; }
  fprintf(stderr, "[k4 stamps] %d workgroups: loads+transforms %.0f, frame sum + eigen %.0f, stores+reduce %.0f cycles (mean per workgroup); last one ends at %.0f cycles\n", n, a / n, e / n, w / n, last);
}

int launch_residual(vba_ctx *c, const double *pd, const int *gate, int head, int end, double *dst = nullptr) {
  double *part = dst ? dst : c->d_partial;
  const int nb = residual_nb(c, end - head);
  static const bool want_stamps = diag_env("VBA_K4_STAMPS") != nullptr;
  static long long *d_st = nullptr;
  if (want_stamps) {
    if (!d_st) hipMalloc((void **)&d_st, 2048 * 4 * 8);
    hipMemsetAsync(d_st, 0, 2048 * 4 * 8, c->stream);
  }
  if (residual_vpl(c, end - head)) {
#define VBA_RESV_CASE(WW) case WW: \
    if (want_stamps) hipLaunchKernelGGL((k_residual_v<WW, true>), dim3(nb), dim3(64), 0, c->stream, c->fv, pd, head, end, part, gate, d_st); \
    else hipLaunchKernelGGL((k_residual_v<WW, false>), dim3(nb), dim3(64), 0, c->stream, c->fv, pd, head, end, part, gate, (long long *)nullptr); break;
    switch (c->opt.win_size) {
      VBA_RESV_CASE(2) VBA_RESV_CASE(3) VBA_RESV_CASE(4) VBA_RESV_CASE(5) VBA_RESV_CASE(6) VBA_RESV_CASE(7) VBA_RESV_CASE(8) VBA_RESV_CASE(9) VBA_RESV_CASE(10)
      VBA_RESV_CASE(11) VBA_RESV_CASE(12) VBA_RESV_CASE(13) VBA_RESV_CASE(14) VBA_RESV_CASE(15) VBA_RESV_CASE(16)
    }
#undef VBA_RESV_CASE
  } else {
#define VBA_RES_CASE(WW) case WW: { using RC = ResCfg<WW, VBA_K4_TV>; \
    if (want_stamps) hipLaunchKernelGGL((k_residual_s<WW, VBA_K4_TV, true>), dim3(nb), dim3(RC::NT), 0, c->stream, c->fv, pd, head, end, part, gate, d_st); \
    else hipLaunchKernelGGL((k_residual_s<WW, VBA_K4_TV, false>), dim3(nb), dim3(RC::NT), 0, c->stream, c->fv, pd, head, end, part, gate, (long long *)nullptr); break; }
    switch (c->opt.win_size) {
      VBA_RES_CASE(2) VBA_RES_CASE(3) VBA_RES_CASE(4) VBA_RES_CASE(5) VBA_RES_CASE(6) VBA_RES_CASE(7) VBA_RES_CASE(8) VBA_RES_CASE(9) VBA_RES_CASE(10)
      VBA_RES_CASE(11) VBA_RES_CASE(12) VBA_RES_CASE(13) VBA_RES_CASE(14) VBA_RES_CASE(15) VBA_RES_CASE(16)
    }
#undef VBA_RES_CASE
  }
  if (want_stamps) k4_stamps_dump(c, nb, d_st);
  return nb;
}

int ctx_allreduce(vba_ctx *c, double *buf, size_t n) {
  if (c->comm) {
    const RcclApi &R = rccl_api();
    const ncclResult_t r = R.AllReduce(buf, buf, n, ncclDouble, ncclSum, c->comm, c->stream);
    if (r != ncclSuccess) { c->set_error(std::string("ncclAllReduce: ") + R.GetErrorString(r)); return VBA_ERR_HIP; }
    return VBA_OK;
  }
  if (!c->allreduce) { c->set_error("no collective configured"); return VBA_ERR_BAD_ARG; }
  if (c->allreduce(c->allreduce_user, buf, n, c->stream)) { c->set_error("allreduce hook failed"); return VBA_ERR_HIP; }
  return VBA_OK;
}
int ctx_allgather(vba_ctx *c, double *buf, size_t chunk) {
  if (chunk == 0) return VBA_OK;
  if (c->comm) {
    const RcclApi &R = rccl_api();
    const ncclResult_t r = R.AllGather(buf + (size_t)c->rank * chunk, buf, chunk, ncclDouble, c->comm, c->stream);
    if (r != ncclSuccess) { c->set_error(std::string("ncclAllGather: ") + R.GetErrorString(r)); return VBA_ERR_HIP; }
    return VBA_OK;
  }
  for (int r = 0; r < c->n_ranks; r++)
    if (r != c->rank) HIPCHK(c, hipMemsetAsync(buf + (size_t)r * chunk, 0, chunk * sizeof(double), c->stream));
  return ctx_allreduce(c, buf, chunk * (size_t)c->n_ranks);
}

int hessian_pass(vba_ctx *c, const double *poses_dev, const int *gate, int head, int end, LmDev *lm = nullptr, const double *k4p = nullptr, int k4nb = 0,
                 const LiJob &li = LiJob{}, size_t li_lds = 0) {
  const int W = c->opt.win_size, nout = nout_tl(W);
  if (end <= head) {
    HIPCHK(c, hipMemsetAsync(c->d_out, 0, (size_t)nout * sizeof(double), c->stream));
  } else {
    int nb = 0;
    TimedSpan s1{}, s2{};
    span_begin(c, "hessian", s1);
    int st = launch_hessian(c, poses_dev, gate, head, end, &nb, lm, k4p, k4nb, li, li_lds);
    if (st) return st;
    span_end(c, "hessian", s1);
    span_begin(c, "reduce", s2);
    hipLaunchKernelGGL(k_reduce_partials, dim3((nout + 15) / 16), dim3(256), 0, c->stream, c->d_partial, nb, nout, c->d_out, gate);
    span_end(c, "reduce", s2);
    HIPCHK(c, hipGetLastError());
  }
  if (c->collective()) {
    int rc = ctx_allreduce(c, c->d_out, (size_t)nout);
    if (rc) return rc;
  }
  return VBA_OK;
}

int residual_pass(vba_ctx *c, const double *poses_dev, const int *gate, int head, int end, double *d_scalar_out) {
  if (end <= head) {
    HIPCHK(c, hipMemsetAsync(d_scalar_out, 0, sizeof(double), c->stream));
  } else {
    const int nb = residual_nb(c, end - head);
    if ((size_t)nb > c->partial_doubles) { c->set_error("partial buffer too small"); return VBA_ERR_CAPACITY; }
    TimedSpan s1{}, s2{};
    span_begin(c, "residual", s1);
    launch_residual(c, poses_dev, gate, head, end);
    span_end(c, "residual", s1);
    span_begin(c, "reduce", s2);
    hipLaunchKernelGGL(k_sum_scalar, dim3(1), dim3(256), 0, c->stream, c->d_partial, nb, d_scalar_out, gate);
    span_end(c, "reduce", s2);
    HIPCHK(c, hipGetLastError());
  }
  if (c->collective()) {
    int rc = ctx_allreduce(c, d_scalar_out, 1);
    if (rc) return rc;
  }
  return VBA_OK;
}

int tiles_to_full(vba_ctx *c, const double *src) {
#define VBA_TF_CASE(WW) case WW: hipLaunchKernelGGL(k_tiles_to_full<WW>, dim3(16), dim3(256), 0, c->stream, src, c->d_full); break;
  switch (c->opt.win_size) {
    VBA_TF_CASE(2) VBA_TF_CASE(3) VBA_TF_CASE(4) VBA_TF_CASE(5) VBA_TF_CASE(6) VBA_TF_CASE(7) VBA_TF_CASE(8) VBA_TF_CASE(9) VBA_TF_CASE(10)
    VBA_TF_CASE(11) VBA_TF_CASE(12) VBA_TF_CASE(13) VBA_TF_CASE(14) VBA_TF_CASE(15) VBA_TF_CASE(16)
    default: return VBA_ERR_UNSUPPORTED_WINDOW;
  }
#undef VBA_TF_CASE
  HIPCHK(c, hipGetLastError());
  return VBA_OK;
}

int eval_hessian_dev(vba_ctx *c, const double *poses, int head, int end) {
  int st = upload_poses(c, poses);
  if (st) return st;
  st = hessian_pass(c, c->d_poses, nullptr, head, end);
  if (st) return st;
  return tiles_to_full(c, c->d_out);
}

int eval_residual_dev(vba_ctx *c, const double *poses, int head, int end, double *d_scalar_out) {
  int st = upload_poses(c, poses);
  if (st) return st;
  return residual_pass(c, c->d_poses, nullptr, head, end, d_scalar_out);
}

int ensure_partial(vba_ctx *c, size_t doubles) {
  if (doubles <= c->partial_doubles) return VBA_OK;
  if (c->d_partial) hipFree(c->d_partial);
  c->d_partial = nullptr; c->partial_doubles = 0;
  HIPCHK(c, hipMalloc((void **)&c->d_partial, doubles * sizeof(double)));
  c->partial_doubles = doubles;
  return VBA_OK;
}

int fetch(vba_ctx *c, const double *d_src, size_t n, double *dst) {
  int st = ensure_pin(c, n + 65536);
  if (st) return st;
  double *stage = c->h_pin + 32768;
  HIPCHK(c, hipStreamSynchronize(c->stream));
  HIPCHK(c, hipMemcpyAsync(stage, d_src, n * sizeof(double), hipMemcpyDeviceToHost, c->stream));
  HIPCHK(c, hipStreamSynchronize(c->stream));
  std::memcpy(dst, stage, n * sizeof(double));
  return VBA_OK;
}

void states_to_poses(const double *states, int W, double *poses) {
  for (int i = 0; i < W; i++) { std::memcpy(poses + 12 * i, states + 25 * i + 1, 9 * sizeof(double)); std::memcpy(poses + 12 * i + 9, states + 25 * i + 10, 3 * sizeof(double)); }
}

}

extern "C" {

void vba_default_options(vba_options *o) {
  std::memset(o, 0, sizeof(*o));
  o->win_size = 10; o->voxel_size = 1.0; o->max_layer = 2; o->max_points = 100; o->min_eigen_value = 0.0025;
  for (int i = 0; i < 4; i++) { o->plane_eigen_value_thre[i] = 0.25; o->min_point[i] = 5; }
  o->imu_coef = 1e-4; o->thread_num = 5; o->device = -1; o->stream = nullptr;
}

const char *vba_status_string(int s) {
  switch (s) {
    case VBA_OK: return "ok";
    case VBA_ERR_NO_DEVICE: return "no HIP device (libvoxelba has no CPU path)";
    case VBA_ERR_BAD_ARG: return "bad argument";
    case VBA_ERR_UNSUPPORTED_WINDOW: return "unsupported window size";
    case VBA_ERR_TOO_FEW_VOXELS: return "too few voxels (reference: 'Too Less Voxel' exit)";
    case VBA_ERR_OPT_STATE: return "opt_state out of range (reference: exit)";
    case VBA_ERR_HIP: return "HIP runtime error";
    case VBA_ERR_CAPACITY: return "capacity exceeded";
    case VBA_ERR_IO: return "file missing or malformed";
    case VBA_ERR_UNSUPPORTED: return "not available in this process (RCCL could not be resolved)";
    case VBA_ERR_SINGULAR: return "singular system (a component without a prior, or a non-positive pivot)";
    default: return "unknown";
  }
}

int vba_create(const vba_options *opt, vba_ctx **out) {
  if (!opt || !out) return VBA_ERR_BAD_ARG;
  *out = nullptr;
  if (opt->win_size < 2 || opt->win_size > VBA_MAX_WIN) return VBA_ERR_UNSUPPORTED_WINDOW;
  int ndev = 0;
  if (hipGetDeviceCount(&ndev) != hipSuccess || ndev <= 0) return VBA_ERR_NO_DEVICE;
  vba_ctx *c = new vba_ctx();
  c->opt = *opt;
  if (opt->device >= 0) {
    if (hipSetDevice(opt->device) != hipSuccess) { delete c; return VBA_ERR_NO_DEVICE; }
    c->device = opt->device;
  } else {
    hipGetDevice(&c->device);
  }
  c->lm_spec = opt->lm_spec > 0 ? std::min(opt->lm_spec, (int)LM_SPEC) : (int)LM_SPEC;
  c->force_collective = opt->force_collective != 0;
  c->max_blocks_hess = opt->hessian_workgroups > 0 ? std::min(opt->hessian_workgroups, kMaxBlocksHess) : kMaxBlocksHess;
  if (c->max_blocks_hess < 2) c->max_blocks_hess = 2;
  c->residual_vpl_from = opt->residual_vpl_from > 0 ? opt->residual_vpl_from : 45000;
  c->use_h3 = opt->hessian_compact_tiles != 0 && opt->deterministic == 0;
  if (opt->stream) { c->stream = (hipStream_t)opt->stream; c->own_stream = false; }
  else {
    if (hipStreamCreateWithFlags(&c->stream, hipStreamNonBlocking) != hipSuccess) { delete c; return VBA_ERR_HIP; }
    c->own_stream = true;
  }
  const int W = opt->win_size, nout = nout_of(W);
  c->fv.W = W;
  if (hipMalloc((void **)&c->d_poses, (size_t)VBA_MAX_WIN * 12 * sizeof(double)) != hipSuccess ||
      hipMalloc((void **)&c->d_out, ((size_t)nout_tl(W) + 64) * sizeof(double)) != hipSuccess ||
      hipMalloc((void **)&c->d_full, ((size_t)nout + 64) * sizeof(double)) != hipSuccess ||
      hipMalloc((void **)&c->d_scal, 64 * sizeof(double)) != hipSuccess) { vba_destroy(c); return VBA_ERR_HIP; }
  if (ensure_partial(c, (size_t)kMaxBlocksHess * (nout_tl(W) > nout ? nout_tl(W) : nout)) != VBA_OK || ensure_pin(c, 65536 + (size_t)nout + 1024) != VBA_OK) { vba_destroy(c); return VBA_ERR_HIP; }
  if (hipMalloc((void **)&c->d_lm, sizeof(LmDev)) != hipSuccess || hipMalloc((void **)&c->d_raw, ((size_t)nout_tl(W) + 64) * 8) != hipSuccess ||
      hipHostMalloc((void **)&c->h_lm, sizeof(LmDev), hipHostMallocDefault) != hipSuccess) { vba_destroy(c); return VBA_ERR_HIP; }
  if (opt->max_voxels && factor_reserve(c, (int)opt->max_voxels) != VBA_OK) { vba_destroy(c); return VBA_ERR_HIP; }
  map_init(c->map, c->opt);
  *out = c;
  return VBA_OK;
}

void vba_destroy(vba_ctx *c) {
  if (!c) return;
  hipSetDevice(c->device);
  if (c->stream) hipStreamSynchronize(c->stream);
  if (c->comm && c->own_comm) rccl_api().CommDestroy(c->comm);
  map_free(c->map);
  c->gba.free_all();
  c->big.release();
  for (vba_ctx *w : c->hba_workers) vba_destroy(w);
  c->hba_workers.clear();
  if (c->d_hba_all) hipFree(c->d_hba_all);
  if (c->d_init) hipFree(c->d_init);
  if (c->d_btcq) hipFree(c->d_btcq);
  if (c->h_btcq) hipHostFree(c->h_btcq);
  if (c->d_btccnt) hipFree(c->d_btccnt);
  if (c->d_icp) hipFree(c->d_icp);
  if (c->h_icp) hipHostFree(c->h_icp);
  if (c->d_icpkey) hipFree(c->d_icpkey);
  if (c->d_icppart) hipFree(c->d_icppart);
  if (c->d_pgo) hipFree(c->d_pgo);
  if (c->d_pgoAb) hipFree(c->d_pgoAb);
  for (int i = 0; i < vba_ctx::kExpRing; i++) { if (c->h_exp[i]) hipHostFree(c->h_exp[i]); if (c->exp_ev[i]) hipEventDestroy(c->exp_ev[i]); }
  if (c->d_exp) hipFree(c->d_exp);
  if (c->d_expout) hipFree(c->d_expout);
  if (c->d_lipack) hipFree(c->d_lipack);
  if (c->d_liscr) hipFree(c->d_liscr);
  for (int i = 0; i < 2; i++) if (c->d_kdtree[i]) hipFree(c->d_kdtree[i]);
  if (c->d_refpts) hipFree(c->d_refpts);
  if (c->d_li) hipFree(c->d_li);
  if (c->d_k4part) hipFree(c->d_k4part);
  if (c->d_imu) hipFree(c->d_imu);
  if (c->d_himu) hipFree(c->d_himu);
  if (c->d_gimu) hipFree(c->d_gimu);
  double *p[] = {c->fv.cl, c->fv.fix, c->fv.coe, c->fv.eigval, c->fv.eigvec, c->fv.pcr, c->d_poses, c->d_partial, c->d_out, c->d_full, c->d_scal};
  for (double *q : p) if (q) hipFree(q);
  if (c->fv.occ) hipFree(c->fv.occ);
  if (c->fv.tiles) hipFree(c->fv.tiles);
  if (c->d_stage) hipFree(c->d_stage);
  if (c->h_pin) hipHostFree(c->h_pin);
  if (c->d_lm) hipFree(c->d_lm);
  if (c->d_raw) hipFree(c->d_raw);
  if (c->h_lm) hipHostFree(c->h_lm);
  for (int i = 0; i < vba_ctx::kLmRing; i++) { if (c->h_lm_up[i]) hipHostFree(c->h_lm_up[i]); if (c->lm_up_ev[i]) hipEventDestroy(c->lm_up_ev[i]); }
  for (auto &kv : c->spans) for (auto &s : kv.second) { hipEventDestroy(s.a); hipEventDestroy(s.b); }
  if (c->own_stream && c->stream) hipStreamDestroy(c->stream);
  delete c;
}

const char *vba_last_error(vba_ctx *c) { return c ? c->err.c_str() : ""; }
int vba_synchronize(vba_ctx *c) { HIPCHK(c, hipStreamSynchronize(c->stream)); return VBA_OK; }

int vba_factor_clear(vba_ctx *c) { c->nvox = 0; return VBA_OK; }
int vba_factor_size(vba_ctx *c) { return c->nvox; }

int vba_factor_push_voxels(vba_ctx *c, int n, const double *clusters, const double *fix, const double *coe, const double *eig_val,
                           const double *eig_vec, const double *pcr_add) {
  if (n < 0) return VBA_ERR_BAD_ARG;
  if (n == 0) return VBA_OK;
  const int W = c->opt.win_size;
  int st = factor_reserve(c, c->nvox + n);
  if (st) return st;
  const size_t per = (size_t)10 * W + 33;
  st = ensure_stage(c, per * n * sizeof(double));
  if (st) return st;
  double *d = (double *)c->d_stage;
  double *d_cl = d, *d_fix = d_cl + (size_t)n * W * 10, *d_coe = d_fix + (size_t)n * 10, *d_ev = d_coe + n, *d_evec = d_ev + (size_t)n * 3,
         *d_pcr = d_evec + (size_t)n * 9;
  HIPCHK(c, hipMemcpyAsync(d_cl, clusters, (size_t)n * W * 10 * sizeof(double), hipMemcpyHostToDevice, c->stream));
  HIPCHK(c, hipMemcpyAsync(d_fix, fix, (size_t)n * 10 * sizeof(double), hipMemcpyHostToDevice, c->stream));
  HIPCHK(c, hipMemcpyAsync(d_coe, coe, (size_t)n * sizeof(double), hipMemcpyHostToDevice, c->stream));
  HIPCHK(c, hipMemcpyAsync(d_ev, eig_val, (size_t)n * 3 * sizeof(double), hipMemcpyHostToDevice, c->stream));
  HIPCHK(c, hipMemcpyAsync(d_evec, eig_vec, (size_t)n * 9 * sizeof(double), hipMemcpyHostToDevice, c->stream));
  HIPCHK(c, hipMemcpyAsync(d_pcr, pcr_add, (size_t)n * 10 * sizeof(double), hipMemcpyHostToDevice, c->stream));
  const long long tot = (long long)n * per;
  int nb = (int)((tot + 255) / 256);
  if (nb > 4096) nb = 4096;
  hipLaunchKernelGGL(k_aos_to_soa, dim3(nb), dim3(256), 0, c->stream, c->fv, c->nvox, n, d_cl, d_fix, d_coe, d_ev, d_evec, d_pcr);
  factor_update_mask(c, c->nvox, n);
  HIPCHK(c, hipGetLastError());
  HIPCHK(c, hipStreamSynchronize(c->stream));
  c->nvox += n;
  return VBA_OK;
}

int vba_factor_acc_evaluate2(vba_ctx *c, const double *poses, int head, int end, double *Hess, double *JacT, double *residual) {
  if (head < 0 || end > c->nvox || head > end) return VBA_ERR_BAD_ARG;
  const int W = c->opt.win_size, n = 6 * W, nout = nout_of(W);
  int st = eval_hessian_dev(c, poses, head, end);
  if (st) return st;
  std::vector<double> buf(nout);
  st = fetch(c, c->d_full, nout, buf.data());
  if (st) return st;
  if (Hess) std::memcpy(Hess, buf.data(), (size_t)n * n * sizeof(double));
  if (JacT) std::memcpy(JacT, buf.data() + (size_t)n * n, (size_t)n * sizeof(double));
  if (residual) *residual = buf[(size_t)n * n + n];
  return VBA_OK;
}

int vba_factor_evaluate_only_residual(vba_ctx *c, const double *poses, int head, int end, double *residual) {
  if (head < 0 || end > c->nvox || head > end) return VBA_ERR_BAD_ARG;
  double *d_r = c->d_scal;
  int st = eval_residual_dev(c, poses, head, end, d_r);
  if (st) return st;
  double r = 0;
  st = fetch(c, d_r, 1, &r);
  if (st) return st;
  if (residual) *residual = r;
  return VBA_OK;
}

int vba_factor_read_back(vba_ctx *c, double *eig_val, double *eig_vec, double *pcr_add) {
  const int n = c->nvox;
  if (n == 0) return VBA_OK;
  int st = ensure_stage(c, (size_t)n * 22 * sizeof(double));
  if (st) return st;
  double *d = (double *)c->d_stage;
  double *d_ev = d, *d_evec = d + (size_t)n * 3, *d_pcr = d_evec + (size_t)n * 9;
  int nb = (int)(((long long)n * 22 + 255) / 256);
  if (nb > 4096) nb = 4096;
  hipLaunchKernelGGL(k_soa_to_aos_out, dim3(nb), dim3(256), 0, c->stream, c->fv, n, d_ev, d_evec, d_pcr);
  HIPCHK(c, hipGetLastError());
  if (eig_val) HIPCHK(c, hipMemcpyAsync(eig_val, d_ev, (size_t)n * 3 * sizeof(double), hipMemcpyDeviceToHost, c->stream));
  if (eig_vec) HIPCHK(c, hipMemcpyAsync(eig_vec, d_evec, (size_t)n * 9 * sizeof(double), hipMemcpyDeviceToHost, c->stream));
  if (pcr_add) HIPCHK(c, hipMemcpyAsync(pcr_add, d_pcr, (size_t)n * 10 * sizeof(double), hipMemcpyDeviceToHost, c->stream));
  HIPCHK(c, hipStreamSynchronize(c->stream));
  return VBA_OK;
}

int vba_factor_occupancy_masks(vba_ctx *c, unsigned int *masks) {
  if (!masks && c->nvox > 0) return VBA_ERR_BAD_ARG;
  if (c->nvox == 0) return VBA_OK;
  HIPCHK(c, hipMemcpyAsync(masks, c->fv.occ, (size_t)c->nvox * sizeof(unsigned int), hipMemcpyDeviceToHost, c->stream));
  HIPCHK(c, hipStreamSynchronize(c->stream));
  return VBA_OK;
}
int vba_factor_occupied_slots(vba_ctx *c, long long *slots) {
  if (!slots) return VBA_ERR_BAD_ARG;
  *slots = 0;
  if (c->nvox == 0) return VBA_OK;
  int st = ensure_stage(c, 64);
  if (st) return st;
  HIPCHK(c, hipMemsetAsync(c->d_stage, 0, 8, c->stream));
  hipLaunchKernelGGL(k_count_slots, dim3(512), dim3(256), 0, c->stream, c->fv, c->nvox, (unsigned long long *)c->d_stage);
  unsigned long long h = 0;
  HIPCHK(c, hipMemcpyAsync(&h, c->d_stage, 8, hipMemcpyDeviceToHost, c->stream));
  HIPCHK(c, hipStreamSynchronize(c->stream));
  *slots = (long long)h;
  return VBA_OK;
}

int vba_lm_begin(vba_ctx *c, const double *poses, int thd_num) {
  const int W = c->opt.win_size;
  const int slot = c->lm_up_next;
  c->lm_up_next = (slot + 1) % vba_ctx::kLmRing;
  if (!c->h_lm_up[slot]) {
    HIPCHK(c, hipHostMalloc((void **)&c->h_lm_up[slot], sizeof(LmDev), hipHostMallocDefault));
    HIPCHK(c, hipEventCreateWithFlags(&c->lm_up_ev[slot], hipEventDisableTiming));
  } else {
    HIPCHK(c, hipEventSynchronize(c->lm_up_ev[slot]));
  }
  LmDev *h = c->h_lm_up[slot];
  std::memset(h, 0, sizeof(LmDev));
  std::memcpy(h->x, poses, (size_t)W * 12 * sizeof(double));
  std::memcpy(h->xt, poses, (size_t)W * 12 * sizeof(double));
  h->u = 0.01; h->v = 2;
  h->is_calc_hess = 1; h->stop = 0; h->iter = 0; h->n_trace = 0; h->all_accepted = 1; h->last_accepted = 0; h->max_trace = 64;
  h->run_hess = 1; h->run_res = 1;
  { const char *e = diag_env("VBA_DEBUG_SOLVE"); h->pad = e ? atoi(e) : 0; }
  HIPCHK(c, hipMemcpyAsync(c->d_lm, h, sizeof(LmDev), hipMemcpyHostToDevice, c->stream));
  HIPCHK(c, hipEventRecord(c->lm_up_ev[slot], c->stream));
  c->lm.active = true; c->lm.thd_num = thd_num; c->lm.have_hess = false; c->lm.pending_update = false;
  c->trace.clear();
  c->nvox_global = c->nvox;
  if (c->collective()) {
    int st = ensure_pin(c, 65536);
    if (st) return st;
    c->h_pin[60000] = (double)c->nvox;
    HIPCHK(c, hipMemcpyAsync(c->d_scal + 8, c->h_pin + 60000, sizeof(double), hipMemcpyHostToDevice, c->stream));
    st = ctx_allreduce(c, c->d_scal + 8, 1);
    if (st) return st;
    HIPCHK(c, hipStreamSynchronize(c->stream));
    HIPCHK(c, hipMemcpyAsync(c->h_pin + 60000, c->d_scal + 8, sizeof(double), hipMemcpyDeviceToHost, c->stream));
    HIPCHK(c, hipStreamSynchronize(c->stream));
    c->nvox_global = (int)(c->h_pin[60000] + 0.5);
  }
  return VBA_OK;
}

int vba_lm_refresh_eigen(vba_ctx *c) {
  if (!c->lm.active) return VBA_ERR_BAD_ARG;
  const double *x_dev = reinterpret_cast<const double *>(reinterpret_cast<char *>(c->d_lm) + offsetof(LmDev, x));
  if (c->nvox <= 0) return VBA_OK;
  if ((size_t)residual_nb(c, c->nvox) > c->partial_doubles) { c->set_error("partial buffer too small"); return VBA_ERR_CAPACITY; }
  TimedSpan s1{};
  span_begin(c, "residual", s1);
  launch_residual(c, x_dev, nullptr, 0, c->nvox);
  span_end(c, "residual", s1);
  HIPCHK(c, hipGetLastError());
  return VBA_OK;
}

int vba_timing_launch_hessian(vba_ctx *c) {
  if (!c->lm.active || c->nvox <= 0) return VBA_ERR_BAD_ARG;
  const double *x_dev = reinterpret_cast<const double *>(reinterpret_cast<char *>(c->d_lm) + offsetof(LmDev, x));
  int nb = 0;
  const int st = launch_hessian(c, x_dev, nullptr, 0, c->nvox, &nb);
  if (st) return st;
  HIPCHK(c, hipGetLastError());
  return VBA_OK;
}

int vba_lm_iterate(vba_ctx *c, int *accepted, int *stop) {
  if (!c->lm.active) return VBA_ERR_BAD_ARG;
  const int W = c->opt.win_size, nout = nout_of(W), V = c->nvox;
  if (c->nvox_global < c->lm.thd_num) return VBA_ERR_TOO_FEW_VOXELS;
  char *base = reinterpret_cast<char *>(c->d_lm);
  const double *x_dev = reinterpret_cast<const double *>(base + offsetof(LmDev, x));
  const double *xt_dev = reinterpret_cast<const double *>(base + offsetof(LmDev, xt));
  const int *run_hess = reinterpret_cast<const int *>(base + offsetof(LmDev, run_hess));
  const int *run_res = reinterpret_cast<const int *>(base + offsetof(LmDev, run_res));
  const int copy_raw = c->collective() ? 1 : 0;
  int st = VBA_OK;
  static const bool no_fuse = diag_env("VBA_NO_FUSED_UPDATE") != nullptr;
  if (!(copy_raw && c->lm.have_hess)) {
    if (c->lm.pending_update) {
      st = hessian_pass(c, x_dev, run_hess, 0, V, c->d_lm, c->d_k4part, c->lm.k4_nb);
      c->lm.pending_update = false;
    } else {
      st = hessian_pass(c, x_dev, run_hess, 0, V);
    }
  }
  if (st) return st;
  TimedSpan sp{};
  span_begin(c, "solve", sp);
  switch (W) {
#define VBA_SM_CASE(WW) case WW: \
    if (copy_raw) hipLaunchKernelGGL((k_lm_solve_m<WW, true>), dim3(c->lm_spec), dim3(256), 0, c->stream, c->d_lm, c->d_out, c->d_raw, nullptr); \
    else hipLaunchKernelGGL((k_lm_solve_m<WW, false>), dim3(c->lm_spec), dim3(256), 0, c->stream, c->d_lm, c->d_out, c->d_raw, nullptr); \
    break;
    VBA_SM_CASE(2) VBA_SM_CASE(3) VBA_SM_CASE(4) VBA_SM_CASE(5) VBA_SM_CASE(6) VBA_SM_CASE(7) VBA_SM_CASE(8) VBA_SM_CASE(9) VBA_SM_CASE(10)
    VBA_SM_CASE(11) VBA_SM_CASE(12) VBA_SM_CASE(13) VBA_SM_CASE(14) VBA_SM_CASE(15) VBA_SM_CASE(16)
#undef VBA_SM_CASE
    default: return VBA_ERR_UNSUPPORTED_WINDOW;
  }
  span_end(c, "solve", sp);
  double *d_r = c->d_scal;
  if (copy_raw) {
    if (V > 0) launch_residual(c, xt_dev, run_res, 0, V);
    st = hessian_pass(c, xt_dev, run_res, 0, V);
    if (st) return st;
    c->lm.have_hess = true;
    hipLaunchKernelGGL(k_lm_update, dim3(1), dim3(64), 0, c->stream, c->d_lm, c->d_out + (nout_tl(W) - 1), 0, W);
  } else {
    const int nb = residual_nb(c, V);
    if (nb > c->k4part_cap) {
      if (c->d_k4part) { HIPCHK(c, hipStreamSynchronize(c->stream)); hipFree(c->d_k4part); c->d_k4part = nullptr; }
      const int cap = nb > 65536 ? 2 * nb : 65536;
      HIPCHK(c, hipMalloc((void **)&c->d_k4part, (size_t)cap * sizeof(double)));
      c->k4part_cap = cap;
    }
    const bool fuse = !no_fuse && !(accepted || stop);
    TimedSpan s1{};
    span_begin(c, "residual", s1);
    launch_residual(c, xt_dev, run_res, 0, V, c->d_k4part);
    span_end(c, "residual", s1);
    if (fuse) { c->lm.pending_update = true; c->lm.k4_nb = nb; }
    else hipLaunchKernelGGL(k_lm_update, dim3(1), dim3(64), 0, c->stream, c->d_lm, c->d_k4part, nb, W);
  }
  HIPCHK(c, hipGetLastError());
  if (accepted || stop) {
    HIPCHK(c, hipMemcpyAsync(c->h_lm, c->d_lm, sizeof(LmDev), hipMemcpyDeviceToHost, c->stream));
    HIPCHK(c, hipStreamSynchronize(c->stream));
    if (accepted) *accepted = c->h_lm->last_accepted;
    if (stop) *stop = c->h_lm->stop;
  }
  return VBA_OK;
}

int vba_lm_end(vba_ctx *c, double *poses, double *hess, double *resis2) {
  if (!c->lm.active) return VBA_ERR_BAD_ARG;
  const int W = c->opt.win_size, n = 6 * W;
  if (c->lm.pending_update) {
    hipLaunchKernelGGL(k_lm_update, dim3(1), dim3(64), 0, c->stream, c->d_lm, c->d_k4part, c->lm.k4_nb, W);
    c->lm.pending_update = false;
  }
  if (!poses && !hess && !resis2) { c->lm.active = false; return VBA_OK; }
  hipLaunchKernelGGL(k_words_to_host, dim3(4), dim3(256), 0, c->stream, (const int *)c->d_lm, (int *)c->h_lm, (int)(sizeof(LmDev) / 4));
  if (hess) {
    int st = ensure_pin(c, 65536 + (size_t)n * n + 1024);
    if (st) return st;
    const double *src = c->collective() ? c->d_raw : c->d_out;
    st = tiles_to_full(c, src);
    if (st) return st;
    hipLaunchKernelGGL(k_words_to_host, dim3(16), dim3(256), 0, c->stream, (const int *)c->d_full, (int *)(c->h_pin + 32768), n * n * 2);
  }
  HIPCHK(c, hipGetLastError());
  HIPCHK(c, hipStreamSynchronize(c->stream));
  const LmDev *h = c->h_lm;
  if (poses) std::memcpy(poses, h->x, (size_t)W * 12 * sizeof(double));
  if (hess) std::memcpy(hess, c->h_pin + 32768, (size_t)n * n * sizeof(double));
  if (resis2) { resis2[0] = h->resis_first; resis2[1] = h->r2; }
  c->trace.assign(h->trace, h->trace + 5 * h->n_trace);
  if (h->pad & 16) {
    fprintf(stderr, "[k_lm_solve_m cycles] prologue %lld | tile load %lld | factorisation %lld | backsub %lld | epilogue %lld | panels:", h->stamps[1] - h->stamps[0],
            h->stamps[2] - h->stamps[1], h->stamps[3] - h->stamps[2], h->stamps[4] - h->stamps[3], h->stamps[5] - h->stamps[4]);
    for (int kb = 0; kb < 8; kb++) fprintf(stderr, " %lld+%lld", h->stamps[9 + 2 * kb] - h->stamps[8 + 2 * kb], kb < 7 ? h->stamps[10 + 2 * kb] - h->stamps[9 + 2 * kb] : 0LL);
    fprintf(stderr, "\n");
  }
  c->lm.active = false;
  return VBA_OK;
}

int vba_lidar_ba_damping_iter(vba_ctx *c, double *poses, double *hess, double *resis2, int max_iter, int thd_num, int *is_converge) {
  int st = vba_lm_begin(c, poses, thd_num);
  if (st) return st;
  for (int i = 0; i < max_iter; i++) {
    st = vba_lm_iterate(c, nullptr, nullptr);
    if (st) { c->lm.active = false; return st; }
  }
  st = vba_lm_end(c, poses, hess, resis2);
  if (is_converge) *is_converge = c->h_lm->all_accepted;
  return st;
}

int vba_last_lm_trace(vba_ctx *c, double *rows, int max_rows) {
  int n = (int)(c->trace.size() / 5);
  if (n > max_rows) n = max_rows;
  if (rows) std::memcpy(rows, c->trace.data(), (size_t)n * 5 * sizeof(double));
  return n;
}

extern "C++" {
template <int W>
struct LiSolveCfg {
  static constexpr int NMAX = 15 * W + 3, NP = ((NMAX + 1 + 15) / 16) * 16;
  static constexpr bool GL = W > 10;
  static constexpr size_t l_doubles = (size_t)LdltCfg<NP>::LTOT > (size_t)NMAX * (NMAX + 1) / 2 ? (size_t)LdltCfg<NP>::LTOT : (size_t)NMAX * (NMAX + 1) / 2;
  static constexpr size_t lds = ((GL ? (size_t)LdltCfg<NP>::DOUBLES - LdltCfg<NP>::LTOT : (size_t)LdltCfg<NP>::DOUBLES) + 4 * NMAX + NP + 32) * 8 + (size_t)NMAX * 4 + 64;
  static_assert(GL || l_doubles == (size_t)LdltCfg<NP>::LTOT, "the staged triangle must fit the region of L");
};
template <int W, int NT = (W > 10 ? 1024 : 512)>
static int launch_li_solve(vba_ctx *c, int copy_raw, int n, int gauge, int grav) {
  constexpr bool GL = LiSolveCfg<W>::GL;
  constexpr size_t l_doubles = LiSolveCfg<W>::l_doubles, lds = LiSolveCfg<W>::lds;
  static bool attr_set[kMaxDevices] = {false};
  if (!attr_set[c->device % kMaxDevices]) { hipFuncSetAttribute((const void *)k_li_solve<W, NT, GL>, hipFuncAttributeMaxDynamicSharedMemorySize, (int)lds); attr_set[c->device % kMaxDevices] = true; }
  if (GL && c->liscr_doubles < l_doubles * LM_SPEC) {
    HIPCHK(c, hipStreamSynchronize(c->stream));
    if (c->d_liscr) hipFree(c->d_liscr);
    c->d_liscr = nullptr; c->liscr_doubles = 0;
    HIPCHK(c, hipMalloc((void **)&c->d_liscr, l_doubles * LM_SPEC * sizeof(double)));
    c->liscr_doubles = l_doubles * LM_SPEC;
  }
  hipLaunchKernelGGL((k_li_solve<W, NT, GL>), dim3(c->lm_spec), dim3(NT), lds, c->stream, c->d_lm, c->d_li, c->d_out, c->d_raw, copy_raw, c->d_himu, c->d_gimu, c->d_imu, n, gauge, grav,
                     c->opt.imu_coef, c->d_liscr, nullptr);
  return VBA_OK;
}
}

static bool li_device_supported(int W) { return W >= 2 && W <= LI_MAX_W; }

static int li_ba_device(vba_ctx *c, double *states, double *imus, int gravity, int max_iter, double *hess, double *resis2) {
  static const bool want_times = diag_env("VBA_LI_TIMES") != nullptr;
  const auto t_0 = std::chrono::steady_clock::now();
  auto since = [&](std::chrono::steady_clock::time_point a) { return std::chrono::duration<double, std::micro>(std::chrono::steady_clock::now() - a).count(); };
  const int W = c->opt.win_size, V = c->nvox, DIM = VBA_DIM, F = W - 1;
  const int n = W * DIM + (gravity ? 3 : 0), nb = gravity ? 33 : 30, n6 = 6 * W;
  if (!gravity) max_iter = 3;
  if (!c->d_li) {
    HIPCHK(c, hipMalloc((void **)&c->d_li, sizeof(LiDev)));
    HIPCHK(c, hipMalloc((void **)&c->d_imu, (size_t)LI_MAX_W * 304 * sizeof(double)));
    HIPCHK(c, hipMalloc((void **)&c->d_himu, (size_t)LI_MAX_N * LI_MAX_N * sizeof(double)));
    HIPCHK(c, hipMalloc((void **)&c->d_gimu, (size_t)LI_MAX_N * sizeof(double)));
  }
  std::vector<double> poses((size_t)W * 12);
  states_to_poses(states, W, poses.data());
  int st = vba_lm_begin(c, poses.data(), 0);
  if (st) return st;
  LiDev h{};
  h.W = W; h.n = n; h.nb = nb; h.gravity = gravity ? 1 : 0; h.gauge = gravity ? 6 : DIM; h.F = F; h.imu_coef = c->opt.imu_coef;
  for (int i = 0; i < W; i++) {
    const double *sx = states + 25 * i;
    h.tstamp[i] = sx[0];
    for (int k = 0; k < 12; k++) h.ex[12 * i + k] = h.ext[12 * i + k] = sx[13 + k];
  }
  std::vector<double> fimg((size_t)F * 304);
  std::memcpy(fimg.data(), imus, fimg.size() * sizeof(double));
  for (int f = 0; f < F; f++) {
    const double *cov = imus + 304 * (size_t)f + 79;
    double *dst = fimg.data() + 304 * (size_t)f + 79;
    bool hit = false;
    for (auto &e : c->covinv_cache)
      if (std::memcmp(e.data(), cov, 225 * sizeof(double)) == 0) { std::memcpy(dst, e.data() + 225, 225 * sizeof(double)); hit = true; break; }
    if (!hit) {
      vbh::inverse_pplu(cov, dst, 15);
      const bool grow = c->covinv_cache.size() < 32;
      if (grow) c->covinv_cache.emplace_back();
      auto &e = grow ? c->covinv_cache.back() : c->covinv_cache[c->covinv_next++ % 32];
      std::memcpy(e.data(), cov, 225 * sizeof(double)); std::memcpy(e.data() + 225, dst, 225 * sizeof(double));
    }
  }
  {
    HIPCHK(c, hipMemcpyAsync(c->d_li, &h, sizeof(LiDev), hipMemcpyHostToDevice, c->stream));
    HIPCHK(c, hipMemcpyAsync(c->d_imu, fimg.data(), fimg.size() * sizeof(double), hipMemcpyHostToDevice, c->stream));
  }
  HIPCHK(c, hipMemsetAsync(c->d_himu, 0, (size_t)li_hb_size(W, 1) * sizeof(double), c->stream));
  HIPCHK(c, hipMemsetAsync(c->d_gimu, 0, (size_t)n * sizeof(double), c->stream));
  char *base = reinterpret_cast<char *>(c->d_lm);
  const double *x_dev = reinterpret_cast<const double *>(base + offsetof(LmDev, x));
  const double *xt_dev = reinterpret_cast<const double *>(base + offsetof(LmDev, xt));
  const int *run_hess = reinterpret_cast<const int *>(base + offsetof(LmDev, run_hess));
  const int *run_res = reinterpret_cast<const int *>(base + offsetof(LmDev, run_res));
  const int copy_raw = c->collective() ? 1 : 0;
  const size_t lds_imu = ((size_t)2 * F * 15 * nb + 2 * F * 15 + F + 16) * sizeof(double);
  {
    static bool attr_set[kMaxDevices] = {false};
    constexpr int FM = LI_MAX_W - 1;
    if (!attr_set[c->device % kMaxDevices]) { hipFuncSetAttribute((const void *)k_li_imu, hipFuncAttributeMaxDynamicSharedMemorySize, (int)(((size_t)2 * FM * 15 * 33 + 2 * FM * 15 + FM + 16) * sizeof(double))); attr_set[c->device % kMaxDevices] = true; }
  }
  const double t_up = since(t_0);
  for (int it = 0; it < max_iter; it++) {
    const bool lidar_now = !(copy_raw && c->lm.have_hess) && V > 0 && lds_imu <= 150 * 1024;
    if (lidar_now) {
      const LiJob job{c->d_lm, c->d_li, c->d_imu, c->d_himu, c->d_gimu};
      st = hessian_pass(c, x_dev, run_hess, 0, V, nullptr, nullptr, 0, job, lds_imu);
    } else {
      hipLaunchKernelGGL(k_li_imu, dim3(1), dim3(LI_IMU_NT), lds_imu, c->stream, c->d_lm, c->d_li, c->d_imu, c->d_himu, c->d_gimu);
      if (!(copy_raw && c->lm.have_hess)) st = hessian_pass(c, x_dev, run_hess, 0, V);
    }
    if (st) { c->lm.active = false; return st; }
    TimedSpan s1{};
    span_begin(c, "solve", s1);
    switch (W) {
      case 2: st = launch_li_solve<2>(c, copy_raw, n, h.gauge, h.gravity); break;
      case 3: st = launch_li_solve<3>(c, copy_raw, n, h.gauge, h.gravity); break;
      case 4: st = launch_li_solve<4>(c, copy_raw, n, h.gauge, h.gravity); break;
      case 5: st = launch_li_solve<5>(c, copy_raw, n, h.gauge, h.gravity); break;
      case 6: st = launch_li_solve<6>(c, copy_raw, n, h.gauge, h.gravity); break;
      case 7: st = launch_li_solve<7>(c, copy_raw, n, h.gauge, h.gravity); break;
      case 9: st = launch_li_solve<9>(c, copy_raw, n, h.gauge, h.gravity); break;
      case 8: st = launch_li_solve<8>(c, copy_raw, n, h.gauge, h.gravity); break;
      case 10: {
        static const int nt = diag_env("VBA_LI_NT") ? atoi(diag_env("VBA_LI_NT")) : 512;
        if (nt == 256) st = launch_li_solve<10, 256>(c, copy_raw, n, h.gauge, h.gravity); else if (nt == 1024) st = launch_li_solve<10, 1024>(c, copy_raw, n, h.gauge, h.gravity); else st = launch_li_solve<10, 512>(c, copy_raw, n, h.gauge, h.gravity);
        break;
      }
      case 11: st = launch_li_solve<11>(c, copy_raw, n, h.gauge, h.gravity); break;
      case 12: st = launch_li_solve<12>(c, copy_raw, n, h.gauge, h.gravity); break;
      case 13: st = launch_li_solve<13>(c, copy_raw, n, h.gauge, h.gravity); break;
      case 14: st = launch_li_solve<14>(c, copy_raw, n, h.gauge, h.gravity); break;
      case 15: st = launch_li_solve<15>(c, copy_raw, n, h.gauge, h.gravity); break;
      case 16: st = launch_li_solve<16>(c, copy_raw, n, h.gauge, h.gravity); break;
      default: c->lm.active = false; return VBA_ERR_UNSUPPORTED_WINDOW;
    }
    span_end(c, "solve", s1);
    if (st) { c->lm.active = false; return st; }
    if (copy_raw) {
      if (V > 0) launch_residual(c, xt_dev, run_res, 0, V);
      st = hessian_pass(c, xt_dev, run_res, 0, V);
      if (st) { c->lm.active = false; return st; }
      c->lm.have_hess = true;
      hipLaunchKernelGGL(k_li_update, dim3(1), dim3(LI_UPD_NT), 0, c->stream, c->d_lm, c->d_li, c->d_imu, c->d_out + (nout_tl(W) - 1), 0);
    } else if (V == 0) {
      st = residual_pass(c, xt_dev, run_res, 0, V, c->d_scal);
      if (st) { c->lm.active = false; return st; }
      hipLaunchKernelGGL(k_li_update, dim3(1), dim3(LI_UPD_NT), 0, c->stream, c->d_lm, c->d_li, c->d_imu, c->d_scal, 0);
    } else {
      const int nbk = residual_nb(c, V);
      TimedSpan s2{};
      span_begin(c, "residual", s2);
      launch_residual(c, xt_dev, run_res, 0, V);
      span_end(c, "residual", s2);
      hipLaunchKernelGGL(k_li_update, dim3(1), dim3(LI_UPD_NT), 0, c->stream, c->d_lm, c->d_li, c->d_imu, c->d_partial, nbk);
    }
    HIPCHK(c, hipGetLastError());
  }
  const double t_enq = since(t_0);
  const double t_gpu = since(t_0);
  static_assert(sizeof(LiDev) % 8 == 0 && sizeof(LmDev) % 8 == 0, "packed as doubles");
  const size_t o_li = 0, o_img = o_li + sizeof(LiDev) / 8, o_hb = o_img + fimg.size(), o_lid = o_hb + (size_t)li_hb_size(W, 1),
               o_lm = o_lid + (size_t)n6 * n6, o_end = o_lm + sizeof(LmDev) / 8;
  st = ensure_pin(c, o_end + 64);
  if (st) return st;
  if (o_end + 64 > c->lipack_doubles) {
    if (c->d_lipack) hipFree(c->d_lipack);
    c->d_lipack = nullptr; c->lipack_doubles = 0;
    HIPCHK(c, hipMalloc((void **)&c->d_lipack, (o_end + 64) * sizeof(double)));
    c->lipack_doubles = o_end + 64;
  }
  PackSegs segs{};
  segs.n = 3;
  segs.src[0] = (const double *)c->d_li; segs.off[0] = o_li; segs.len[0] = sizeof(LiDev) / 8;
  segs.src[1] = c->d_imu; segs.off[1] = o_img; segs.len[1] = fimg.size();
  segs.src[2] = (const double *)c->d_lm; segs.off[2] = o_lm; segs.len[2] = sizeof(LmDev) / 8;
  if (hess) {
    st = tiles_to_full(c, copy_raw ? c->d_raw : c->d_out);
    if (st) return st;
    segs.n = 5;
    segs.src[3] = c->d_full; segs.off[3] = o_lid; segs.len[3] = (size_t)n6 * n6;
    segs.src[4] = c->d_himu; segs.off[4] = o_hb; segs.len[4] = (size_t)li_hb_size(W, gravity);
  }
  hipLaunchKernelGGL(k_pack_segments, dim3(64, segs.n), dim3(256), 0, c->stream, segs, c->d_lipack);
  HIPCHK(c, hipGetLastError());
  HIPCHK(c, hipMemcpyAsync(c->h_pin, c->d_lipack, o_end * sizeof(double), hipMemcpyDeviceToHost, c->stream));
  HIPCHK(c, hipStreamSynchronize(c->stream));
  std::memcpy(c->h_lm, c->h_pin + o_lm, sizeof(LmDev));
  std::memcpy(&h, c->h_pin + o_li, sizeof(LiDev));
  std::memcpy(fimg.data(), c->h_pin + o_img, fimg.size() * sizeof(double));
  const double *himu_h = c->h_pin + o_hb;
  c->lm.active = false;
  const LmDev *hl = c->h_lm;
  for (int i = 0; i < W; i++) {
    double *sx = states + 25 * i;
    for (int k = 0; k < 12; k++) sx[1 + k] = hl->x[12 * i + k];
    for (int k = 0; k < 12; k++) sx[13 + k] = h.ex[12 * i + k];
  }
  if (hl->use_spec)
    for (int f = 0; f < F; f++) std::memcpy(fimg.data() + 304 * (size_t)f + 67, fimg.data() + 304 * (size_t)f + 73, 6 * sizeof(double));
  for (int f = 0; f < F; f++) std::memcpy(imus + 304 * (size_t)f + 67, fimg.data() + 304 * (size_t)f + 67, 12 * sizeof(double));
  if (hess) {
    const double *lid = c->h_pin + o_lid;
    for (int r = 0; r < n; r++)
      for (int k = 0; k < n; k++) hess[(size_t)r * n + k] = c->opt.imu_coef * li_hb_get(himu_h, W, n, r, k);
    for (int i = 0; i < W; i++)
      for (int j = 0; j < W; j++)
        for (int r = 0; r < 6; r++)
          for (int k = 0; k < 6; k++) hess[(size_t)(i * DIM + r) * n + j * DIM + k] += lid[(size_t)(i * 6 + r) * n6 + j * 6 + k];
  }
  if (gravity && resis2) { resis2[0] = hl->resis_first; resis2[1] = hl->r2; }
  c->trace.assign(hl->trace, hl->trace + 5 * hl->n_trace);
  if (want_times && (hl->pad & 16)) {
    fprintf(stderr, "[k_li_solve prologue] stage imu %lld | stage lidar %lld | diag+g %lld | rank %lld\n", hl->stamps[50] - hl->stamps[0], hl->stamps[51] - hl->stamps[50], hl->stamps[52] - hl->stamps[51], hl->stamps[1] - hl->stamps[52]);
    fprintf(stderr, "[k_li_solve cycles] prologue %lld | tile load %lld | factorisation %lld | backsub %lld | epilogue %lld | panels:", hl->stamps[1] - hl->stamps[0],
            hl->stamps[2] - hl->stamps[1], hl->stamps[3] - hl->stamps[2], hl->stamps[4] - hl->stamps[3], hl->stamps[5] - hl->stamps[4]);
    for (int kb = 0; kb < 20; kb++) fprintf(stderr, " %lld+%lld", hl->stamps[9 + 2 * kb] - hl->stamps[8 + 2 * kb], kb < 19 ? hl->stamps[10 + 2 * kb] - hl->stamps[9 + 2 * kb] : 0LL);
    fprintf(stderr, "\n");
  }
  if (want_times && (hl->pad & 64)) fprintf(stderr, "[k_li_imu cycles] factor algebra (one lane per factor) %lld | cov^-1 joc %lld | contractions %lld\n", hl->stamps[41] - hl->stamps[40], hl->stamps[42] - hl->stamps[41], hl->stamps[43] - hl->stamps[42]);
  if (want_times && (hl->pad & 32)) { double v[6]; std::memcpy(v, &hl->stamps[58], sizeof(v)); fprintf(stderr, "[li r1 parts] rank %d: rimu %.10g lidar %.10g | %.10g %.10g | %.10g %.10g\n", c->rank, v[0], v[1], v[2], v[3], v[4], v[5]); }
  if (want_times) fprintf(stderr, "[li_ba_device] upload %.1f us | enqueue %.1f | gpu drained at %.1f | total %.1f\n", t_up, t_enq - t_up, t_gpu, since(t_0));
  return VBA_OK;
}

int vba_li_ba_damping_iter(vba_ctx *c, double *states, double *imus, int gravity, int max_iter, double *hess, double *resis2) {
  if (!li_device_supported(c->opt.win_size)) return VBA_ERR_UNSUPPORTED_WINDOW;
  return li_ba_device(c, states, imus, gravity, max_iter, hess, resis2);
}

static int kd_reserve(vba_ctx *c, size_t pts) {
  if (pts <= c->kd_cap) return VBA_OK;
  size_t cap = c->kd_cap ? c->kd_cap : 65536;
  while (cap < pts) cap *= 2;
  for (int i = 0; i < 2; i++) {
    double *nw = nullptr;
    HIPCHK(c, hipMalloc((void **)&nw, cap * 3 * sizeof(double)));
    if (c->d_kdtree[i]) {
      if (i == c->kd_cur && c->kd_n > 0) HIPCHK(c, hipMemcpyAsync(nw, c->d_kdtree[i], (size_t)c->kd_n * 3 * sizeof(double), hipMemcpyDeviceToDevice, c->stream));
      HIPCHK(c, hipStreamSynchronize(c->stream));
      hipFree(c->d_kdtree[i]);
    }
    c->d_kdtree[i] = nw;
  }
  c->kd_cap = cap;
  return VBA_OK;
}
int vba_odom_kdtree_reset(vba_ctx *c) { c->kd_n = 0; return VBA_OK; }
int vba_odom_kdtree_size(vba_ctx *c) { return c->kd_n; }
int vba_odom_kdtree_points(vba_ctx *c, double *out) {
  if (!out && c->kd_n > 0) return VBA_ERR_BAD_ARG;
  if (c->kd_n == 0) return VBA_OK;
  HIPCHK(c, hipStreamSynchronize(c->stream));
  HIPCHK(c, hipMemcpyAsync(out, c->d_kdtree[c->kd_cur], (size_t)c->kd_n * 3 * sizeof(double), hipMemcpyDefault, c->stream));
  HIPCHK(c, hipStreamSynchronize(c->stream));
  return VBA_OK;
}

int vba_odom_lio_state_estimation_kdtree(vba_ctx *c, int n, const double *pnt_body, double *state, double *cov, int *iterations) {
  if (n < 0 || (n > 0 && !pnt_body) || !state || !cov) return VBA_ERR_BAD_ARG;
  if (iterations) *iterations = 0;
  const int DIM = VBA_DIM, nb = (n + 255) / 256;
  const int kd_slices = nb >= 512 ? 1 : (nb >= 128 ? 4 : 8);
  int st = ensure_stage(c, ((size_t)n * 7 + (size_t)nb * 28 + (size_t)kd_slices * n * 5 + 64) * sizeof(double));
  if (st) return st;
  double *d_pts = (double *)c->d_stage, *d_pl = d_pts + (size_t)n * 3, *d_part = d_pl + (size_t)n * 4;
  unsigned long long *d_cand = (unsigned long long *)(d_part + (size_t)nb * 28);
  if (n > 0) HIPCHK(c, hipMemcpyAsync(d_pts, pnt_body, (size_t)n * 3 * sizeof(double), hipMemcpyDefault, c->stream));
  vbh::State x_curr, x_prop;
  std::memcpy(&x_curr, state, sizeof(x_curr));
  auto pose_of = [](const vbh::State &x) { KdPose X; std::memcpy(X.R, x.R, sizeof(X.R)); std::memcpy(X.t, x.p, sizeof(X.t)); return X; };
  st = kd_reserve(c, (size_t)c->kd_n + (size_t)n + 16);
  if (st) return st;
  if (c->kd_n < 100) {
    if (n > 0) hipLaunchKernelGGL(k_kd_append, dim3(nb), dim3(256), 0, c->stream, n, d_pts, pose_of(x_curr), c->d_kdtree[c->kd_cur] + (size_t)c->kd_n * 3);
    HIPCHK(c, hipGetLastError());
    HIPCHK(c, hipStreamSynchronize(c->stream));
    c->kd_n += n;
    return VBA_OK;
  }
  x_prop = x_curr;
  std::vector<double> P(cov, cov + 225), cov_inv(225), part((size_t)nb * 28);
  vbh::inverse_pplu(P.data(), cov_inv.data(), DIM);
  const int num_max_iter = 4;
  int rematch_num = 0, iters = 0;
  bool refind = true, converged_once = false;
  double G[225];
  std::memset(G, 0, sizeof(G));
  for (int iter = 0; iter < num_max_iter; iter++) {
    iters++;
    const KdPose X = pose_of(x_curr);
    double s28[28];
    std::memset(s28, 0, sizeof(s28));
    if (n > 0) {
      if (refind) {
        hipLaunchKernelGGL(k_kd_match, dim3(nb, kd_slices), dim3(256), 0, c->stream, n, d_pts, X, c->kd_n, c->d_kdtree[c->kd_cur], d_cand);
        hipLaunchKernelGGL(k_kd_fit, dim3(nb), dim3(256), 0, c->stream, n, kd_slices, d_cand, c->d_kdtree[c->kd_cur], d_pl);
      }
      hipLaunchKernelGGL(k_kd_accum, dim3(nb), dim3(256), 0, c->stream, n, d_pts, X, d_pl, d_part);
      HIPCHK(c, hipGetLastError());
      HIPCHK(c, hipStreamSynchronize(c->stream));
      HIPCHK(c, hipMemcpyAsync(part.data(), d_part, part.size() * sizeof(double), hipMemcpyDeviceToHost, c->stream));
      HIPCHK(c, hipStreamSynchronize(c->stream));
      for (int b = 0; b < nb; b++) for (int k = 0; k < 28; k++) s28[k] += part[(size_t)b * 28 + k];
    }
    double HTH[36], HTz[6];
    { int idx = 0; for (int r = 0; r < 6; r++) for (int k = r; k < 6; k++) { HTH[r * 6 + k] = s28[idx]; HTH[k * 6 + r] = s28[idx]; idx++; } }
    for (int r = 0; r < 6; r++) HTz[r] = s28[21 + r];
    std::vector<double> A(225), K1(225);
    for (int k = 0; k < 225; k++) A[k] = cov_inv[k] / 1000;
    for (int r = 0; r < 6; r++) for (int k = 0; k < 6; k++) A[r * DIM + k] += HTH[r * 6 + k];
    vbh::inverse_pplu(A.data(), K1.data(), DIM);
    for (int r = 0; r < DIM; r++)
      for (int k = 0; k < 6; k++) { double sacc = 0; for (int j = 0; j < 6; j++) sacc += K1[r * DIM + j] * HTH[j * 6 + k]; G[r * DIM + k] = sacc; }
    double vec[15], RtR[9], lg[3];
    vbh::m3_Tmul(x_curr.R, x_prop.R, RtR);
    vbh::so3_log(RtR, lg);
    for (int k = 0; k < 3; k++) { vec[k] = lg[k]; vec[3 + k] = x_prop.p[k] - x_curr.p[k]; vec[6 + k] = x_prop.v[k] - x_curr.v[k]; vec[9 + k] = x_prop.bg[k] - x_curr.bg[k]; vec[12 + k] = x_prop.ba[k] - x_curr.ba[k]; }
    double sol[15];
    for (int r = 0; r < DIM; r++) {
      double a = 0, b = 0;
      for (int j = 0; j < 6; j++) { a += K1[r * DIM + j] * HTz[j]; b += G[r * DIM + j] * vec[j]; }
      sol[r] = a + vec[r] - b;
    }
    double E[9], Rn[9];
    vbh::so3_exp(sol, E);
    vbh::m3_mul(x_curr.R, E, Rn);
    std::memcpy(x_curr.R, Rn, sizeof(Rn));
    for (int k = 0; k < 3; k++) { x_curr.p[k] += sol[3 + k]; x_curr.v[k] += sol[6 + k]; x_curr.bg[k] += sol[9 + k]; x_curr.ba[k] += sol[12 + k]; }
    const double rot_add = vbh::norm3(sol), tra_add = vbh::norm3(sol + 3);
    refind = false;
    if ((rot_add * 57.3 < 0.01) && (tra_add * 100 < 0.015)) { refind = true; converged_once = true; rematch_num++; }
    if (iter == num_max_iter - 2 && !converged_once) refind = true;
    if (rematch_num >= 2 || (iter == num_max_iter - 1)) {
      std::vector<double> IG(225), Pn(225);
      for (int r = 0; r < DIM; r++) for (int k = 0; k < DIM; k++) IG[r * DIM + k] = (r == k ? 1.0 : 0.0) - G[r * DIM + k];
      vbh::mat_mul(IG.data(), P.data(), Pn.data(), DIM, DIM, DIM);
      P = Pn;
      break;
    }
  }
  if (n > 0) hipLaunchKernelGGL(k_kd_append, dim3(nb), dim3(256), 0, c->stream, n, d_pts, pose_of(x_curr), c->d_kdtree[c->kd_cur] + (size_t)c->kd_n * 3);
  HIPCHK(c, hipGetLastError());
  HIPCHK(c, hipStreamSynchronize(c->stream));
  const int tot = c->kd_n + n;
  {
    std::vector<int> cnt(tot), first(tot);
    int m = 0;
    st = vba_scan_down_sampling_voxel(c, tot, c->d_kdtree[c->kd_cur], 0.5, c->d_kdtree[c->kd_cur ^ 1], cnt.data(), first.data(), &m);
    if (st) return st;
    c->kd_cur ^= 1; c->kd_n = m;
  }
  std::memcpy(state, &x_curr, sizeof(x_curr));
  std::memcpy(cov, P.data(), 225 * sizeof(double));
  if (iterations) *iterations = iters;
  return VBA_OK;
}

static GbaParams gba_params(vba_ctx *c, double voxel_size, double min_eig, const double *eig_array) {
  GbaParams P;
  P.voxel_size = voxel_size; P.min_eigen_value = min_eig; P.max_layer = c->opt.max_layer;
  for (int k = 0; k < 4; k++) P.eig_array[k] = eig_array[k];
// ... 3188 lines not shown
```

Baseline: 21460.

## Fuse LM state initialization into first kernel and merge end-of-solve readback kernels

Drops the host-side pinned ring buffer and the H2D memcpy of the LM state at lm_begin. The initial poses are now passed by value as a kernel argument, and block 0 of the first residual or hessian kernel writes the LM state image to device memory. A standalone init kernel is used as a fallback where fusion does not apply. At lm_end, the pending update, the state readback and the Hessian tile-to-full copy are merged into one k_lm_finish kernel, cutting launches and copies per solve at the cost of larger kernel arguments and more complex ordering logic.

```diff
diff --git a/voxel-slam_amd/csrc/vba_kernels_factor.hpp b/voxel-slam_amd/csrc/vba_kernels_factor.hpp
--- a/voxel-slam_amd/csrc/vba_kernels_factor.hpp
+++ b/voxel-slam_amd/csrc/vba_kernels_factor.hpp
@@ -222,6 +222,16 @@
   return x;
 }
 
+struct LmDev;
+template <int W>
+struct LmInit {
+  double x[12 * W];
+  LmDev *dst;
+  int on, dbg;
+};
+template <int W>
+__device__ __forceinline__ void lm_init_store(const LmInit<W> &a, int tid, int nt);
+
 template <int W, int TV>
 struct ResCfg {
   static constexpr int NT = ((TV * W + 63) / 64) * 64;
@@ -234,7 +244,7 @@
 template <int W, int TV, bool STAMPS>
 __global__ __launch_bounds__((ResCfg<W, TV>::NT)) void k_residual_s(FactorView f, const double *__restrict__ poses, int head, int end,
                                                                   double *__restrict__ partial, const int *__restrict__ gate,
-                                                                  long long *__restrict__ stamps) {
+                                                                  long long *__restrict__ stamps, LmInit<W> init) {
   using C = ResCfg<W, TV>;
   __shared__ double T[10][W][TV];
   __shared__ double S[10][TV];
@@ -248,7 +258,7 @@
   long long st0 = 0, st1 = 0, st2 = 0, st3 = 0;
   if (STAMPS) st0 = clock64();
   const unsigned int occm = f.occ[vc];
-  const double pose_s = poses[tid < W * 12 ? tid : 0];
+  const double pose_s = init.on ? init.x[tid < W * 12 ? tid : 0] : poses[tid < W * 12 ? tid : 0];
   double acc[C::KPT];
 #pragma unroll
   for (int j = 0; j < C::KPT; j++) { const int k = fi + j * C::NF; acc[j] = f.fix[(size_t)(k < 10 ? k : 9) * vs + vc]; }
@@ -256,6 +266,7 @@
   unsigned int occv = occm;
   asm volatile("" : "+v"(occv), "+v"(coe), "+v"(acc[0]));
   if (gate_v == 0) return;
+  if (init.on && blockIdx.x == 0) lm_init_store(init, tid, C::NT);
   if (tid < W * 12) sp[tid] = pose_s;
   const bool occ = fi < W && v < end && ((occv >> fic) & 1u);
   double c[9], n = 0.0;
@@ -313,9 +324,10 @@
   }
 }
 
-template <int W, bool STAMPS>
+template <int W, bool STAMPS, bool INIT = false>
 __global__ __launch_bounds__(64) void k_residual_v(FactorView f, const double *__restrict__ poses, int head, int end,
-                                                   double *__restrict__ partial, const int *__restrict__ gate, long long *__restrict__ stamps) {
+                                                   double *__restrict__ partial, const int *__restrict__ gate, long long *__restrict__ stamps,
+                                                   LmInit<W> init) {
   const int gate_v = gate ? *gate : 1;
   const int lane = threadIdx.x;
   const int v = head + blockIdx.x * 64 + lane;
@@ -330,6 +342,7 @@
   double coe = f.coe[vc];
   asm volatile("" : "+v"(occm), "+v"(coe), "+v"(acc[0]));
   if (gate_v == 0) return;
+  if (INIT && blockIdx.x == 0) lm_init_store(init, lane, 64);
   if (v >= end) occm = 0;
   double c[W][10];
 #pragma unroll
@@ -348,7 +361,7 @@
     const bool on = (occm >> i) & 1u;
     if (__ballot(on) != 0ull) {
       if (on) {
-        const Cl10 w = cluster_transform_exact(c[i][0], c[i][1], c[i][2], c[i][3], c[i][4], c[i][5], c[i][6], c[i][7], c[i][8], c[i][9], poses + 12 * i);
+        const Cl10 w = cluster_transform_exact(c[i][0], c[i][1], c[i][2], c[i][3], c[i][4], c[i][5], c[i][6], c[i][7], c[i][8], c[i][9], (INIT ? init.x : poses) + 12 * i);
         acc[0] += w.p00; acc[1] += w.p10; acc[2] += w.p20; acc[3] += w.p11; acc[4] += w.p21; acc[5] += w.p22;
         acc[6] += w.v0; acc[7] += w.v1; acc[8] += w.v2; acc[9] += w.n;
       }
@@ -385,7 +398,7 @@
 __global__ __launch_bounds__(256) void k_reduce_partials(const double *__restrict__ partial, int nb, int nout, double *__restrict__ out,
                                                         const int *__restrict__ gate) {
   __shared__ double s[256];
-  const int gate_v = gate ? *gate : 1;
+  if (gate && *gate == 0) return;
   const int j = threadIdx.x & 15, q = threadIdx.x >> 4;
   const int o = blockIdx.x * 16 + j, oc = o < nout ? o : nout - 1;
   double pv[16];
@@ -393,7 +406,6 @@
   for (int k = 0; k < 16; k++) { const int b = q + 16 * k; pv[k] = partial[(size_t)(b < nb ? b : 0) * nout + oc]; }
 #pragma unroll
   for (int k = 0; k < 16; k++) asm volatile("" : "+v"(pv[k]));
-  if (gate_v == 0) return;
   double acc = 0.0;
   if (o < nout) {
 #pragma unroll
@@ -582,7 +594,7 @@
 __global__ __launch_bounds__(HessCfg2<W>::NT) void k_hessian2(FactorView f, const double *__restrict__ poses, int head, int end,
                                                              int ntiles, double *__restrict__ partial, const int *__restrict__ gate,
                                                              long long *__restrict__ stamps, LmDev *lm, const double *__restrict__ k4_partial, int k4_nb,
-                                                             int nwg, LiJob li) {
+                                                             int nwg, LiJob li, LmInit<W> init) {
   using C = HessCfg2<W>;
   extern __shared__ __attribute__((aligned(16))) double lds[];
   if (li.dev && blockIdx.x == 0) {
@@ -595,7 +607,7 @@
   unsigned int occ_nx = 0;
   if (my_fi < W && tile0 < tile1) { const int v0 = head + tile0 * HessCfg2<W>::TV + my_vl; occ_nx = f.occ[v0 < end ? v0 : end - 1]; }
   __shared__ int lm_dec[2];
-  int gate_v = (gate && !lm) ? *gate : 1;
+  int gate_v = (gate && !lm && !init.on) ? *gate : 1;
   double lm_r2 = 0.0;
   if (lm) {
     if (threadIdx.x < 64) {
@@ -618,7 +630,12 @@
   double *sp = cK + C::NK;
   const int tid = threadIdx.x, lane = tid & 63, wv = tid >> 6;
 
-  for (int t = tid; t < W * 12; t += C::NT) sp[t] = poses[t];
+  if (init.on) {
+    for (int t = tid; t < W * 12; t += C::NT) sp[t] = init.x[t];
+    if (bid == 0) lm_init_store(init, tid, C::NT);
+  } else {
+    for (int t = tid; t < W * 12; t += C::NT) sp[t] = poses[t];
+  }
   constexpr int PADC = C::GS - C::NC;
   if constexpr (PADC > 0)
     for (int t = tid; t < C::NK * PADC; t += C::NT) { G[(size_t)(t / PADC) * C::GS + C::NC + t % PADC] = 0.0; if (C::PRESCALE) GA[(size_t)(t / PADC) * C::GS + C::NC + t % PADC] = 0.0; }
diff --git a/voxel-slam_amd/csrc/vba_kernels_lm.hpp b/voxel-slam_amd/csrc/vba_kernels_lm.hpp
--- a/voxel-slam_amd/csrc/vba_kernels_lm.hpp
+++ b/voxel-slam_amd/csrc/vba_kernels_lm.hpp
@@ -17,6 +17,30 @@
   double q1_spec[LM_SPEC];
   double xt_spec[LM_SPEC][VBA_MAX_WIN_DEV * 12];
 };
+
+template <int W>
+__device__ __forceinline__ void lm_init_store(const LmInit<W> &a, int tid, int nt) {
+  constexpr int NW = sizeof(LmDev) / 8, XT = offsetof(LmDev, xt) / 8, U = offsetof(LmDev, u) / 8, V = offsetof(LmDev, v) / 8,
+                I = offsetof(LmDev, is_calc_hess) / 8;
+  static_assert(sizeof(LmDev) % 8 == 0 && offsetof(LmDev, x) == 0 && offsetof(LmDev, u) == 2 * offsetof(LmDev, xt) && 12 * W <= XT, "x and xt lead the image");
+  static_assert(offsetof(LmDev, is_calc_hess) % 8 == 0 && offsetof(LmDev, pad) == offsetof(LmDev, is_calc_hess) + 36, "the ten flags are five words");
+  auto two = [](int lo, int hi) { return (unsigned long long)(unsigned int)lo | ((unsigned long long)(unsigned int)hi << 32); };
+  unsigned long long *o = reinterpret_cast<unsigned long long *>(a.dst);
+  for (int w = tid; w < NW; w += nt) {
+    unsigned long long val = 0ull;
+    if (w < 2 * XT) { const int k = w < XT ? w : w - XT; if (k < 12 * W) val = (unsigned long long)__double_as_longlong(a.x[k]); }
+    else if (w == U) val = (unsigned long long)__double_as_longlong(0.01);
+    else if (w == V) val = (unsigned long long)__double_as_longlong(2.0);
+    else if (w == I) val = two(1, 0);
+    else if (w == I + 2) val = two(1, 0);
+    else if (w == I + 3) val = two(64, 1);
+    else if (w == I + 4) val = two(1, a.dbg);
+    o[w] = val;
+  }
+}
+
+template <int W>
+__global__ __launch_bounds__(256) void k_lm_init(LmInit<W> a) { lm_init_store(a, threadIdx.x, 256); }
 
 __device__ __forceinline__ void so3_exp_dev(const double *w, double *R) {
   const double n = sqrt(w[0] * w[0] + w[1] * w[1] + w[2] * w[2]);
@@ -271,4 +295,24 @@
   lm_update_apply(s, r2, W);
 }
 
-}
+template <int W>
+__global__ __launch_bounds__(256) void k_lm_finish(LmDev *s, const double *__restrict__ r2_dev, int nb, int upd, LmDev *h_lm,
+                                                   const double *__restrict__ red, double *__restrict__ h_hess) {
+  if (blockIdx.x == 0) {
+    if (upd && threadIdx.x < 64) {
+      const int stop = s->stop;
+      const double r2 = lm_sum_partials(r2_dev, nb, threadIdx.x);
+      if (!stop) lm_update_apply(s, r2, W);
+      __threadfence();
+    }
+    __syncthreads();
+    const unsigned long long *src = reinterpret_cast<const unsigned long long *>(s);
+    unsigned long long *dst = reinterpret_cast<unsigned long long *>(h_lm);
+    for (int w = threadIdx.x; w < (int)(sizeof(LmDev) / 8); w += 256) dst[w] = __hip_atomic_load(src + w, __ATOMIC_RELAXED, __HIP_MEMORY_SCOPE_AGENT);
+  } else {
+    constexpr int n = 6 * W;
+    for (int t = (blockIdx.x - 1) * 256 + threadIdx.x; t < n * n; t += (gridDim.x - 1) * 256) h_hess[t] = tl_fetch<W>(red, t / n, t % n);
+  }
+}
+
+}
diff --git a/voxel-slam_amd/csrc/voxelba.hip b/voxel-slam_amd/csrc/voxelba.hip
--- a/voxel-slam_amd/csrc/voxelba.hip
+++ b/voxel-slam_amd/csrc/voxelba.hip
@@ -135,10 +135,7 @@
 
   LmDev *d_lm = nullptr;
   LmDev *h_lm = nullptr;
-  static const int kLmRing = 8;
-  LmDev *h_lm_up[kLmRing] = {nullptr};
-  hipEvent_t lm_up_ev[kLmRing] = {nullptr};
-  int lm_up_next = 0;
+  struct { bool pending = false; int dbg = 0; double x[VBA_MAX_WIN_DEV * 12]; } lm_init;
   double *d_raw = nullptr;
   struct { bool active = false; int thd_num = 2; bool have_hess = false; bool pending_update = false; int k4_nb = 0; } lm;
   int k4part_cap = 0;
@@ -268,8 +265,31 @@
 }
 
 template <int W>
+LmInit<W> lm_init_arg(vba_ctx *c, bool take) {
+  LmInit<W> a{};
+  if (take && c->lm_init.pending) {
+    std::memcpy(a.x, c->lm_init.x, sizeof(a.x));
+    a.dst = c->d_lm; a.on = 1; a.dbg = c->lm_init.dbg;
+    c->lm_init.pending = false;
+  }
+  return a;
+}
+int lm_init_flush(vba_ctx *c) {
+  if (!c->lm_init.pending) return VBA_OK;
+  switch (c->opt.win_size) {
+#define VBA_LI_CASE(WW) case WW: hipLaunchKernelGGL(k_lm_init<WW>, dim3(1), dim3(256), 0, c->stream, lm_init_arg<WW>(c, true)); break;
+    VBA_LI_CASE(2) VBA_LI_CASE(3) VBA_LI_CASE(4) VBA_LI_CASE(5) VBA_LI_CASE(6) VBA_LI_CASE(7) VBA_LI_CASE(8) VBA_LI_CASE(9) VBA_LI_CASE(10)
+    VBA_LI_CASE(11) VBA_LI_CASE(12) VBA_LI_CASE(13) VBA_LI_CASE(14) VBA_LI_CASE(15) VBA_LI_CASE(16)
+#undef VBA_LI_CASE
+    default: return VBA_ERR_UNSUPPORTED_WINDOW;
+  }
+  HIPCHK(c, hipGetLastError());
+  return VBA_OK;
+}
+
+template <int W>
 int launch_hessian2_t(vba_ctx *c, const double *poses_dev, const int *gate, int head, int end, int *nblocks_out, LmDev *lm, const double *k4p, int k4nb,
-                      const LiJob &li, size_t li_lds) {
+                      const LiJob &li, size_t li_lds, bool init) {
   using C = HessCfg2<W>;
   const int ntiles = (end - head + C::TV - 1) / C::TV;
   const int maxb = li.dev ? c->max_blocks_hess - 1 : c->max_blocks_hess;
@@ -291,7 +311,7 @@
   }
   const size_t lds = (li.dev && li_lds > C::LDS_BYTES) ? li_lds : C::LDS_BYTES;
   hipLaunchKernelGGL(k_hessian2<W>, dim3(nb + (li.dev ? 1 : 0)), dim3(C::NT), lds, c->stream, c->fv, poses_dev, head, end, ntiles, c->d_partial, gate, stamps, lm, k4p, k4nb,
-                     nb, li);
+                     nb, li, lm_init_arg<W>(c, init));
   if (want_stamps) {
     std::vector<long long> h((size_t)nb * 16);
     hipStreamSynchronize(c->stream);
@@ -351,8 +371,9 @@
 }
 
 int launch_hessian(vba_ctx *c, const double *pd, const int *gate, int head, int end, int *nb, LmDev *lm = nullptr, const double *k4p = nullptr, int k4nb = 0,
-                   const LiJob &li = LiJob{}, size_t li_lds = 0) {
+                   const LiJob &li = LiJob{}, size_t li_lds = 0, bool init = false) {
   if (head == 0 && end == c->nvox && c->opt.win_size <= 10 && c->use_h3) {
+    if (init) { const int st = lm_init_flush(c); if (st) return st; }
     switch (c->opt.win_size) {
 #define VBA_H3_CASE(WW) case WW: return launch_hessian3_t<WW>(c, pd, gate, nb, lm, k4p, k4nb, li, li_lds);
       VBA_H3_CASE(2) VBA_H3_CASE(3) VBA_H3_CASE(4) VBA_H3_CASE(5) VBA_H3_CASE(6) VBA_H3_CASE(7) VBA_H3_CASE(8) VBA_H3_CASE(9) VBA_H3_CASE(10)
@@ -360,7 +381,7 @@
     }
   }
   switch (c->opt.win_size) {
-#define VBA_H_CASE(WW) case WW: return launch_hessian2_t<WW>(c, pd, gate, head, end, nb, lm, k4p, k4nb, li, li_lds);
+#define VBA_H_CASE(WW) case WW: return launch_hessian2_t<WW>(c, pd, gate, head, end, nb, lm, k4p, k4nb, li, li_lds, init);
     VBA_H_CASE(2) VBA_H_CASE(3) VBA_H_CASE(4) VBA_H_CASE(5) VBA_H_CASE(6) VBA_H_CASE(7) VBA_H_CASE(8) VBA_H_CASE(9) VBA_H_CASE(10)
     VBA_H_CASE(11) VBA_H_CASE(12) VBA_H_CASE(13) VBA_H_CASE(14) VBA_H_CASE(15) VBA_H_CASE(16)
 #undef VBA_H_CASE
@@ -386,7 +407,7 @@
   fprintf(stderr, "[k4 stamps] %d workgroups: loads+transforms %.0f, frame sum + eigen %.0f, stores+reduce %.0f cycles (mean per workgroup); last one ends at %.0f cycles\n", n, a / n, e / n, w / n, last);
 }
 
-int launch_residual(vba_ctx *c, const double *pd, const int *gate, int head, int end, double *dst = nullptr) {
+int launch_residual(vba_ctx *c, const double *pd, const int *gate, int head, int end, double *dst = nullptr, bool init = false) {
   double *part = dst ? dst : c->d_partial;
   const int nb = residual_nb(c, end - head);
   static const bool want_stamps = diag_env("VBA_K4_STAMPS") != nullptr;
@@ -395,10 +416,15 @@
     if (!d_st) hipMalloc((void **)&d_st, 2048 * 4 * 8);
     hipMemsetAsync(d_st, 0, 2048 * 4 * 8, c->stream);
   }
+  if (want_stamps && init) {
+    if (lm_init_flush(c)) return -1;
+    init = false;
+  }
   if (residual_vpl(c, end - head)) {
 #define VBA_RESV_CASE(WW) case WW: \
-    if (want_stamps) hipLaunchKernelGGL((k_residual_v<WW, true>), dim3(nb), dim3(64), 0, c->stream, c->fv, pd, head, end, part, gate, d_st); \
-    else hipLaunchKernelGGL((k_residual_v<WW, false>), dim3(nb), dim3(64), 0, c->stream, c->fv, pd, head, end, part, gate, (long long *)nullptr); break;
+    if (want_stamps) hipLaunchKernelGGL((k_residual_v<WW, true>), dim3(nb), dim3(64), 0, c->stream, c->fv, pd, head, end, part, gate, d_st, lm_init_arg<WW>(c, false)); \
+    else if (init && c->lm_init.pending) hipLaunchKernelGGL((k_residual_v<WW, false, true>), dim3(nb), dim3(64), 0, c->stream, c->fv, pd, head, end, part, gate, (long long *)nullptr, lm_init_arg<WW>(c, true)); \
+    else hipLaunchKernelGGL((k_residual_v<WW, false>), dim3(nb), dim3(64), 0, c->stream, c->fv, pd, head, end, part, gate, (long long *)nullptr, lm_init_arg<WW>(c, false)); break;
     switch (c->opt.win_size) {
       VBA_RESV_CASE(2) VBA_RESV_CASE(3) VBA_RESV_CASE(4) VBA_RESV_CASE(5) VBA_RESV_CASE(6) VBA_RESV_CASE(7) VBA_RESV_CASE(8) VBA_RESV_CASE(9) VBA_RESV_CASE(10)
       VBA_RESV_CASE(11) VBA_RESV_CASE(12) VBA_RESV_CASE(13) VBA_RESV_CASE(14) VBA_RESV_CASE(15) VBA_RESV_CASE(16)
@@ -406,8 +432,8 @@
 #undef VBA_RESV_CASE
   } else {
 #define VBA_RES_CASE(WW) case WW: { using RC = ResCfg<WW, VBA_K4_TV>; \
-    if (want_stamps) hipLaunchKernelGGL((k_residual_s<WW, VBA_K4_TV, true>), dim3(nb), dim3(RC::NT), 0, c->stream, c->fv, pd, head, end, part, gate, d_st); \
-    else hipLaunchKernelGGL((k_residual_s<WW, VBA_K4_TV, false>), dim3(nb), dim3(RC::NT), 0, c->stream, c->fv, pd, head, end, part, gate, (long long *)nullptr); break; }
+    if (want_stamps) hipLaunchKernelGGL((k_residual_s<WW, VBA_K4_TV, true>), dim3(nb), dim3(RC::NT), 0, c->stream, c->fv, pd, head, end, part, gate, d_st, lm_init_arg<WW>(c, init)); \
+    else hipLaunchKernelGGL((k_residual_s<WW, VBA_K4_TV, false>), dim3(nb), dim3(RC::NT), 0, c->stream, c->fv, pd, head, end, part, gate, (long long *)nullptr, lm_init_arg<WW>(c, init)); break; }
     switch (c->opt.win_size) {
       VBA_RES_CASE(2) VBA_RES_CASE(3) VBA_RES_CASE(4) VBA_RES_CASE(5) VBA_RES_CASE(6) VBA_RES_CASE(7) VBA_RES_CASE(8) VBA_RES_CASE(9) VBA_RES_CASE(10)
       VBA_RES_CASE(11) VBA_RES_CASE(12) VBA_RES_CASE(13) VBA_RES_CASE(14) VBA_RES_CASE(15) VBA_RES_CASE(16)
@@ -443,15 +469,16 @@
 }
 
 int hessian_pass(vba_ctx *c, const double *poses_dev, const int *gate, int head, int end, LmDev *lm = nullptr, const double *k4p = nullptr, int k4nb = 0,
-                 const LiJob &li = LiJob{}, size_t li_lds = 0) {
+                 const LiJob &li = LiJob{}, size_t li_lds = 0, bool init = false) {
   const int W = c->opt.win_size, nout = nout_tl(W);
   if (end <= head) {
+    if (init) { const int st = lm_init_flush(c); if (st) return st; }
     HIPCHK(c, hipMemsetAsync(c->d_out, 0, (size_t)nout * sizeof(double), c->stream));
   } else {
     int nb = 0;
     TimedSpan s1{}, s2{};
     span_begin(c, "hessian", s1);
-    int st = launch_hessian(c, poses_dev, gate, head, end, &nb, lm, k4p, k4nb, li, li_lds);
+    int st = launch_hessian(c, poses_dev, gate, head, end, &nb, lm, k4p, k4nb, li, li_lds, init);
     if (st) return st;
     span_end(c, "hessian", s1);
     span_begin(c, "reduce", s2);
@@ -648,7 +675,6 @@
   if (c->d_lm) hipFree(c->d_lm);
   if (c->d_raw) hipFree(c->d_raw);
   if (c->h_lm) hipHostFree(c->h_lm);
-  for (int i = 0; i < vba_ctx::kLmRing; i++) { if (c->h_lm_up[i]) hipHostFree(c->h_lm_up[i]); if (c->lm_up_ev[i]) hipEventDestroy(c->lm_up_ev[i]); }
   for (auto &kv : c->spans) for (auto &s : kv.second) { hipEventDestroy(s.a); hipEventDestroy(s.b); }
   if (c->own_stream && c->stream) hipStreamDestroy(c->stream);
   delete c;
@@ -758,24 +784,9 @@
 
 int vba_lm_begin(vba_ctx *c, const double *poses, int thd_num) {
   const int W = c->opt.win_size;
-  const int slot = c->lm_up_next;
-  c->lm_up_next = (slot + 1) % vba_ctx::kLmRing;
-  if (!c->h_lm_up[slot]) {
-    HIPCHK(c, hipHostMalloc((void **)&c->h_lm_up[slot], sizeof(LmDev), hipHostMallocDefault));
-    HIPCHK(c, hipEventCreateWithFlags(&c->lm_up_ev[slot], hipEventDisableTiming));
-  } else {
-    HIPCHK(c, hipEventSynchronize(c->lm_up_ev[slot]));
-  }
-  LmDev *h = c->h_lm_up[slot];
-  std::memset(h, 0, sizeof(LmDev));
-  std::memcpy(h->x, poses, (size_t)W * 12 * sizeof(double));
-  std::memcpy(h->xt, poses, (size_t)W * 12 * sizeof(double));
-  h->u = 0.01; h->v = 2;
-  h->is_calc_hess = 1; h->stop = 0; h->iter = 0; h->n_trace = 0; h->all_accepted = 1; h->last_accepted = 0; h->max_trace = 64;
-  h->run_hess = 1; h->run_res = 1;
-  { const char *e = diag_env("VBA_DEBUG_SOLVE"); h->pad = e ? atoi(e) : 0; }
-  HIPCHK(c, hipMemcpyAsync(c->d_lm, h, sizeof(LmDev), hipMemcpyHostToDevice, c->stream));
-  HIPCHK(c, hipEventRecord(c->lm_up_ev[slot], c->stream));
+  std::memcpy(c->lm_init.x, poses, (size_t)W * 12 * sizeof(double));
+  { const char *e = diag_env("VBA_DEBUG_SOLVE"); c->lm_init.dbg = e ? atoi(e) : 0; }
+  c->lm_init.pending = true;
   c->lm.active = true; c->lm.thd_num = thd_num; c->lm.have_hess = false; c->lm.pending_update = false;
   c->trace.clear();
   c->nvox_global = c->nvox;
@@ -801,7 +812,9 @@
   if ((size_t)residual_nb(c, c->nvox) > c->partial_doubles) { c->set_error("partial buffer too small"); return VBA_ERR_CAPACITY; }
   TimedSpan s1{};
   span_begin(c, "residual", s1);
-  launch_residual(c, x_dev, nullptr, 0, c->nvox);
+  const bool fuse_init = !c->collective();
+  if (!fuse_init) { const int st = lm_init_flush(c); if (st) return st; }
+  if (launch_residual(c, x_dev, nullptr, 0, c->nvox, nullptr, fuse_init) < 0) return VBA_ERR_HIP;
   span_end(c, "residual", s1);
   HIPCHK(c, hipGetLastError());
   return VBA_OK;
@@ -811,7 +824,9 @@
   if (!c->lm.active || c->nvox <= 0) return VBA_ERR_BAD_ARG;
   const double *x_dev = reinterpret_cast<const double *>(reinterpret_cast<char *>(c->d_lm) + offsetof(LmDev, x));
   int nb = 0;
-  const int st = launch_hessian(c, x_dev, nullptr, 0, c->nvox, &nb);
+  int st = lm_init_flush(c);
+  if (st) return st;
+  st = launch_hessian(c, x_dev, nullptr, 0, c->nvox, &nb);
   if (st) return st;
   HIPCHK(c, hipGetLastError());
   return VBA_OK;
@@ -820,7 +835,7 @@
 int vba_lm_iterate(vba_ctx *c, int *accepted, int *stop) {
   if (!c->lm.active) return VBA_ERR_BAD_ARG;
   const int W = c->opt.win_size, nout = nout_of(W), V = c->nvox;
-  if (c->nvox_global < c->lm.thd_num) return VBA_ERR_TOO_FEW_VOXELS;
+  if (c->nvox_global < c->lm.thd_num) { c->lm_init.pending = false; return VBA_ERR_TOO_FEW_VOXELS; }
   char *base = reinterpret_cast<char *>(c->d_lm);
   const double *x_dev = reinterpret_cast<const double *>(base + offsetof(LmDev, x));
   const double *xt_dev = reinterpret_cast<const double *>(base + offsetof(LmDev, xt));
@@ -829,12 +844,13 @@
   const int copy_raw = c->collective() ? 1 : 0;
   int st = VBA_OK;
   static const bool no_fuse = diag_env("VBA_NO_FUSED_UPDATE") != nullptr;
+  if (copy_raw) { st = lm_init_flush(c); if (st) return st; }
   if (!(copy_raw && c->lm.have_hess)) {
     if (c->lm.pending_update) {
       st = hessian_pass(c, x_dev, run_hess, 0, V, c->d_lm, c->d_k4part, c->lm.k4_nb);
       c->lm.pending_update = false;
     } else {
-      st = hessian_pass(c, x_dev, run_hess, 0, V);
+      st = hessian_pass(c, x_dev, run_hess, 0, V, nullptr, nullptr, 0, LiJob{}, 0, true);
     }
   }
   if (st) return st;
@@ -887,20 +903,32 @@
 int vba_lm_end(vba_ctx *c, double *poses, double *hess, double *resis2) {
   if (!c->lm.active) return VBA_ERR_BAD_ARG;
   const int W = c->opt.win_size, n = 6 * W;
-  if (c->lm.pending_update) {
+  const bool want = poses || hess || resis2;
+  if (!want && !c->lm.pending_update) { c->lm_init.pending = false; c->lm.active = false; return VBA_OK; }
+  int st = lm_init_flush(c);
+  if (st) return st;
+  if (!want) {
     hipLaunchKernelGGL(k_lm_update, dim3(1), dim3(64), 0, c->stream, c->d_lm, c->d_k4part, c->lm.k4_nb, W);
     c->lm.pending_update = false;
-  }
-  if (!poses && !hess && !resis2) { c->lm.active = false; return VBA_OK; }
-  hipLaunchKernelGGL(k_words_to_host, dim3(4), dim3(256), 0, c->stream, (const int *)c->d_lm, (int *)c->h_lm, (int)(sizeof(LmDev) / 4));
+    c->lm.active = false;
+    return VBA_OK;
+  }
+  double *h_hess = nullptr;
   if (hess) {
-    int st = ensure_pin(c, 65536 + (size_t)n * n + 1024);
+    st = ensure_pin(c, 65536 + (size_t)n * n + 1024);
     if (st) return st;
-    const double *src = c->collective() ? c->d_raw : c->d_out;
-    st = tiles_to_full(c, src);
-    if (st) return st;
-    hipLaunchKernelGGL(k_words_to_host, dim3(16), dim3(256), 0, c->stream, (const int *)c->d_full, (int *)(c->h_pin + 32768), n * n * 2);
-  }
+    h_hess = c->h_pin + 32768;
+  }
+  const double *src = c->collective() ? c->d_raw : c->d_out;
+  const int upd = c->lm.pending_update ? 1 : 0;
+  switch (W) {
+#define VBA_FIN_CASE(WW) case WW: hipLaunchKernelGGL(k_lm_finish<WW>, dim3(hess ? 17 : 1), dim3(256), 0, c->stream, c->d_lm, c->d_k4part, upd ? c->lm.k4_nb : 0, upd, c->h_lm, src, h_hess); break;
+    VBA_FIN_CASE(2) VBA_FIN_CASE(3) VBA_FIN_CASE(4) VBA_FIN_CASE(5) VBA_FIN_CASE(6) VBA_FIN_CASE(7) VBA_FIN_CASE(8) VBA_FIN_CASE(9) VBA_FIN_CASE(10)
+    VBA_FIN_CASE(11) VBA_FIN_CASE(12) VBA_FIN_CASE(13) VBA_FIN_CASE(14) VBA_FIN_CASE(15) VBA_FIN_CASE(16)
+#undef VBA_FIN_CASE
+    default: return VBA_ERR_UNSUPPORTED_WINDOW;
+  }
+  c->lm.pending_update = false;
   HIPCHK(c, hipGetLastError());
   HIPCHK(c, hipStreamSynchronize(c->stream));
   const LmDev *h = c->h_lm;
@@ -983,6 +1011,8 @@
   std::vector<double> poses((size_t)W * 12);
   states_to_poses(states, W, poses.data());
   int st = vba_lm_begin(c, poses.data(), 0);
+  if (st) return st;
+  st = lm_init_flush(c);
   if (st) return st;
   LiDev h{};
   h.W = W; h.n = n; h.nb = nb; h.gravity = gravity ? 1 : 0; h.gauge = gravity ? 6 : DIM; h.F = F; h.imu_coef = c->opt.imu_coef;
```

Result: faster. 22520 (median of 6 runs) (+5.0%).
